# Kaixhin/imitation-learning

Measured on NVIDIA H100. Metric: env_steps_per_s, higher is better.
Workload: dtype f32

## Files before the change

imitation-learning_b200/csrc/api.cu:

```cuda
#include "common.cuh"
#include <cstdlib>

thread_local char g_il_error[512] = "";
int gail_init();
int gmmil_pwil_init();
int gemm_init();
int mlp_init();

extern "C" const char* il_last_error(void) { return g_il_error; }
extern "C" int il_version(void) { return 100; }

extern "C" int il_create(int device, il_handle** out) {
  IL_CHECK(out != nullptr, "il_create: null out");
  int count = 0;
  cudaError_t e = cudaGetDeviceCount(&count);
  if (e != cudaSuccess || count == 0) IL_FAIL("il_create: no CUDA device (%s); this library has no CPU fallback", cudaGetErrorString(e));
  IL_CHECK(device >= 0 && device < count, "il_create: device %d out of range (%d devices)", device, count);
  cudaDeviceProp prop;
  IL_CUDA(cudaGetDeviceProperties(&prop, device));
  IL_CHECK(prop.major == 9 && prop.minor == 0, "il_create: device %d is sm_%d%d; this library is built for sm_90a (H100) only", device, prop.major, prop.minor);
  IL_CUDA(cudaSetDevice(device));
  IL_TRY(gail_init());
  IL_TRY(gmmil_pwil_init());
  IL_TRY(tc_gemm_init());
  IL_TRY(gemm_init());
  IL_TRY(mlp_init());
  il_handle* h = new il_handle();
  h->device = device;
  h->sm_count = prop.multiProcessorCount;
  h->gemm_mode = IL_GEMM_FP32;
  {
    const char* wt = getenv("IL_WIDE_TN");
    h->wide_tn = (wt && wt[0] == '0') ? 0 : 1;
    const char* ff = getenv("IL_FIRST_LAYER_FAST");
    h->first_layer_fast = ff ? atoi(ff) : 2;
    const char* mb = getenv("IL_MASK_BITS");
    h->mask_bits = mb ? atoi(mb) : 2;
    const char* hf = getenv("IL_HEAD_FUSED");
    h->head_fused = (hf && hf[0] == '0') ? 0 : 1;
    const char* ds = getenv("IL_DEBUG_SYNC");
    h->debug_sync = (ds && ds[0] == '1') ? 1 : 0;
    const char* at = getenv("IL_ADAM_TMA");
    h->adam_tma = at ? atoi(at) : 1;
    const char* gt = getenv("IL_GAIL_TILED");
    h->gail_tiled = (gt && gt[0] == '0') ? 0 : 1;
    const char* fl = getenv("IL_TC_FUSE_L1");
    h->tc_fuse_l1 = (fl && fl[0] == '1') ? 1 : 0;
    const char* th = getenv("IL_THIN_HOIST");
    h->thin_hoist = (th && th[0] == '0') ? 0 : 1;
  }
  h->launches = 0;
  h->profiling = 0;
  h->profiled_bytes = 0.0;
  h->eval_graph = nullptr;
  h->build_stream = nullptr;
  *out = h;
  return 0;
}

extern "C" int il_destroy(il_handle* h) {
  if (h) il_eval_release(h);
  if (h && h->build_stream) cudaStreamDestroy(h->build_stream);
  delete h;
  return 0;
}

extern "C" int il_set_gemm_mode(il_handle* h, int mode) {
  IL_CHECK(h, "il_set_gemm_mode: null handle");
  IL_CHECK(mode >= IL_GEMM_FP32 && mode <= IL_GEMM_TF32, "il_set_gemm_mode: bad mode %d", mode);
  h->gemm_mode = mode;
  return 0;
}

extern "C" int64_t il_launch_count(il_handle* h) { return h ? h->launches : -1; }

extern "C" int il_set_option(il_handle* h, const char* name, int value) {
  IL_CHECK(h && name, "il_set_option: null argument");
  if (!strcmp(name, "tc_fuse_l1")) h->tc_fuse_l1 = value;
  else if (!strcmp(name, "gail_tiled")) h->gail_tiled = value;
  else if (!strcmp(name, "adam_tma")) h->adam_tma = value;
  else if (!strcmp(name, "head_fused")) h->head_fused = value;
  else if (!strcmp(name, "mask_bits")) h->mask_bits = value;
  else if (!strcmp(name, "first_layer_fast")) h->first_layer_fast = value;
  else if (!strcmp(name, "wide_tn")) h->wide_tn = value;
  else if (!strcmp(name, "thin_hoist")) h->thin_hoist = value;
  else IL_FAIL("il_set_option: unknown option '%s'", name);
  return 0;
}

extern "C" int il_struct_sizes(int32_t* out) {
  out[0] = (int32_t)sizeof(il_mlp);
  out[1] = (int32_t)sizeof(il_adam);
  out[2] = (int32_t)sizeof(il_batch);
  out[3] = (int32_t)sizeof(il_replay);
  out[4] = (int32_t)sizeof(il_sac_args);
  out[5] = (int32_t)sizeof(il_gail);
  out[6] = (int32_t)sizeof(il_gail_update_args);
  out[7] = (int32_t)sizeof(il_pwil);
  out[8] = (int32_t)sizeof(il_env);
  out[9] = (int32_t)sizeof(il_bc_args);
  out[10] = (int32_t)sizeof(il_eval_args);
  out[11] = (int32_t)sizeof(il_gailx);
  out[12] = (int32_t)sizeof(il_gailx_update_args);
  out[13] = (int32_t)sizeof(il_red);
  out[14] = (int32_t)sizeof(il_red_update_args);
  return 0;
}

extern "C" int il_mlp_param_offsets(const int32_t* dims, int n_layers, int64_t* w_off, int64_t* b_off, int64_t* total) {
  IL_CHECK(dims && n_layers >= 1 && n_layers <= IL_MAX_LAYERS, "il_mlp_param_offsets: bad arguments");
  const MlpOffsets o = mlp_offsets(dims, n_layers);
  for (int l = 0; l < n_layers; ++l) {
    if (w_off) w_off[l] = o.w[l];
    if (b_off) b_off[l] = o.b[l];
  }
  if (total) *total = o.total;
  return 0;
}

extern "C" int il_row_layout(int S, int A, int32_t* off, int32_t* row_len) {
  IL_CHECK(S > 0 && A > 0, "il_row_layout: S=%d A=%d", S, A);
  const RowLayout L = row_layout(S, A);
  if (off) {
    off[0] = L.state; off[1] = L.action; off[2] = L.reward; off[3] = L.next_state;
    off[4] = L.terminal; off[5] = L.timeout; off[6] = L.weight; off[7] = L.step;
  }
  if (row_len) *row_len = L.len;
  return 0;
}

namespace {

__global__ void fill_kernel(float* __restrict__ out, int64_t n, uint64_t seed, uint64_t stream_id, const uint64_t* __restrict__ counter, int normal,
                            const uint64_t* __restrict__ seed_r) {
  const uint64_t base = counter ? *counter : 0ull;
  if (seed_r) { seed = seed_r[blockIdx.y]; out += (int64_t)blockIdx.y * n; }
  const uint2 key = make_uint2((uint32_t)seed, (uint32_t)(seed >> 32));
  for (int64_t q = (int64_t)blockIdx.x * blockDim.x + threadIdx.x; q * 4 < n; q += (int64_t)gridDim.x * blockDim.x) {
    const uint64_t c = base + (uint64_t)q;
    const uint4 r = philox4x32_10(make_uint4((uint32_t)c, (uint32_t)(c >> 32), (uint32_t)stream_id, (uint32_t)(stream_id >> 32)), key);
    float v[4];
    if (normal) {
      const float u0 = 1.f - u32_to_unit(r.x), u1 = u32_to_unit(r.y), u2 = 1.f - u32_to_unit(r.z), u3 = u32_to_unit(r.w);
      const float r0 = sqrtf(-2.f * logf(u0)), r1 = sqrtf(-2.f * logf(u2));
      float s0, c0, s1, c1;
      sincospif(2.f * u1, &s0, &c0);
      sincospif(2.f * u3, &s1, &c1);
      v[0] = r0 * c0; v[1] = r0 * s0; v[2] = r1 * c1; v[3] = r1 * s1;
    } else {
      v[0] = u32_to_unit(r.x); v[1] = u32_to_unit(r.y); v[2] = u32_to_unit(r.z); v[3] = u32_to_unit(r.w);
    }
    for (int j = 0; j < 4; ++j)
      if (q * 4 + j < n) out[q * 4 + j] = v[j];
  }
}

constexpr int BETA_ATTEMPTS = 16;

__device__ float log_gamma_mt(float a, uint64_t c, uint64_t stream_id, uint32_t tag, uint2 key, float* boost_u) {
  const float d = a - 1.f / 3.f, cc = 1.f / sqrtf(9.f * d);
  for (int k = 0; k < BETA_ATTEMPTS; ++k) {
    const uint4 q = philox4x32_10(make_uint4((uint32_t)c, (uint32_t)(c >> 32), (uint32_t)stream_id, (uint32_t)(stream_id >> 32) ^ (tag | (uint32_t)k)), key);
    if (k == 0) *boost_u = 1.f - u32_to_unit(q.w);
    const float x = sqrtf(-2.f * logf(1.f - u32_to_unit(q.x))) * cospif(2.f * u32_to_unit(q.y));
    const float t = fmaf(cc, x, 1.f);
    if (t <= 0.f) continue;
    const float lt = logf(t), v = t * t * t;
    if (logf(1.f - u32_to_unit(q.z)) < 0.5f * x * x + d - d * v + 3.f * d * lt) return logf(d) + 3.f * lt;
  }
  return logf(d);
}

__global__ void beta_fill_kernel(float* __restrict__ out, int64_t total, int64_t n, const float* __restrict__ alpha_r, uint64_t seed, uint64_t stream_id,
                                 const uint64_t* __restrict__ counter, const uint64_t* __restrict__ seed_r) {
  const uint64_t base = counter ? *counter : 0ull;
  if (seed_r) { seed = seed_r[blockIdx.y]; out += (int64_t)blockIdx.y * n; total = n; }
  const uint2 key = make_uint2((uint32_t)seed, (uint32_t)(seed >> 32));
  for (int64_t i = (int64_t)blockIdx.x * blockDim.x + threadIdx.x; i < total; i += (int64_t)gridDim.x * blockDim.x) {
    const uint64_t c = base + (uint64_t)(i >> 2);
    const uint32_t lane = (uint32_t)(i & 3);
    const float alpha = alpha_r[seed_r ? (int64_t)blockIdx.y : i / n];
    float v;
    if (alpha == 1.f) {
      const uint4 q = philox4x32_10(make_uint4((uint32_t)c, (uint32_t)(c >> 32), (uint32_t)stream_id, (uint32_t)(stream_id >> 32)), key);
      v = u32_to_unit(lane == 0 ? q.x : lane == 1 ? q.y : lane == 2 ? q.z : q.w);
    } else if (!(alpha > 0.f)) {
      v = __int_as_float(0x7fc00000);
    } else {
      const float a = alpha < 1.f ? alpha + 1.f : alpha;
      float ux, uy;
      float lx = log_gamma_mt(a, c, stream_id, 0x80000000u | (lane << 5), key, &ux);
      float ly = log_gamma_mt(a, c, stream_id, 0x80000000u | (lane << 5) | 16u, key, &uy);
      if (alpha < 1.f) { lx += logf(ux) / alpha; ly += logf(uy) / alpha; }
      const float t = ly - lx;
      v = t >= 0.f ? 1.f / (1.f + expf(t)) : 1.f - 1.f / (1.f + expf(-t));
    }
    out[i] = v;
  }
}

__global__ void counter_add_kernel(uint64_t* c, uint64_t inc) { *c += inc; }

dim3 rng_grid(il_handle* h, int64_t units, int R) {
  int64_t blocks = (units + 255) / 256;
  const int64_t cap = (int64_t)h->sm_count * 16 / R;
  if (blocks > cap) blocks = cap;
  if (blocks < 1) blocks = 1;
  return dim3((unsigned)blocks, (unsigned)R);
}

int fill(il_handle* h, float* out, int64_t n, uint64_t seed, uint64_t stream_id, const uint64_t* counter, void* stream, int normal) {
  IL_CHECK(h && out && n >= 0, "il_fill: bad argument");
  if (n == 0) return 0;
  int64_t blocks = (n / 4 + 255) / 256;
  if (blocks > (int64_t)h->sm_count * 16) blocks = (int64_t)h->sm_count * 16;
  if (blocks < 1) blocks = 1;
  IL_LAUNCH(h, fill_kernel, (unsigned)blocks, 256, 0, (cudaStream_t)stream, out, n, seed, stream_id, counter, normal, nullptr);
  return 0;
}

int fill_r(il_handle* h, float* out, int R, int64_t n_per_replica, const uint64_t* seed_r, uint64_t stream_id, const uint64_t* counter, void* stream, int normal) {
  IL_CHECK(h && out && seed_r && R > 0 && R <= IL_MAX_GRID_Y && n_per_replica >= 0, "il_fill_%s_r: bad argument (R = %d)", normal ? "normal" : "uniform", R);
  if (n_per_replica == 0) return 0;
  IL_LAUNCH(h, fill_kernel, rng_grid(h, (n_per_replica + 3) / 4, R), 256, 0, (cudaStream_t)stream, out, n_per_replica, 0ull, stream_id, counter, normal, seed_r);
  return 0;
}

}

extern "C" int il_fill_normal(il_handle* h, float* out, int64_t n, uint64_t seed, uint64_t stream_id, const uint64_t* counter, void* stream) {
  return fill(h, out, n, seed, stream_id, counter, stream, 1);
}
extern "C" int il_fill_uniform(il_handle* h, float* out, int64_t n, uint64_t seed, uint64_t stream_id, const uint64_t* counter, void* stream) {
  return fill(h, out, n, seed, stream_id, counter, stream, 0);
}
extern "C" int il_fill_normal_r(il_handle* h, float* out, int R, int64_t n_per_replica, const uint64_t* seed_r, uint64_t stream_id, const uint64_t* counter, void* stream) {
  return fill_r(h, out, R, n_per_replica, seed_r, stream_id, counter, stream, 1);
}
extern "C" int il_fill_uniform_r(il_handle* h, float* out, int R, int64_t n_per_replica, const uint64_t* seed_r, uint64_t stream_id, const uint64_t* counter, void* stream) {
  return fill_r(h, out, R, n_per_replica, seed_r, stream_id, counter, stream, 0);
}
extern "C" int il_fill_beta(il_handle* h, float* out, int R, int64_t n_per_replica, const float* alpha_r, uint64_t seed, uint64_t stream_id, const uint64_t* counter,
                            void* stream) {
  IL_CHECK(h && out && alpha_r && R > 0 && n_per_replica >= 0, "il_fill_beta: bad argument");
  const int64_t total = (int64_t)R * n_per_replica;
  if (total == 0) return 0;
  int64_t blocks = (total + 255) / 256;
  if (blocks > (int64_t)h->sm_count * 16) blocks = (int64_t)h->sm_count * 16;
  IL_LAUNCH(h, beta_fill_kernel, (unsigned)blocks, 256, 0, (cudaStream_t)stream, out, total, n_per_replica, alpha_r, seed, stream_id, counter, nullptr);
  return 0;
}
extern "C" int il_fill_beta_r(il_handle* h, float* out, int R, int64_t n_per_replica, const float* alpha_r, const uint64_t* seed_r, uint64_t stream_id,
                              const uint64_t* counter, void* stream) {
  IL_CHECK(h && out && alpha_r && seed_r && R > 0 && R <= IL_MAX_GRID_Y && n_per_replica >= 0, "il_fill_beta_r: bad argument (R = %d)", R);
  if (n_per_replica == 0) return 0;
  IL_LAUNCH(h, beta_fill_kernel, rng_grid(h, n_per_replica, R), 256, 0, (cudaStream_t)stream, out, n_per_replica, n_per_replica, alpha_r, 0ull, stream_id, counter, seed_r);
  return 0;
}
extern "C" int il_counter_add(il_handle* h, uint64_t* counter, uint64_t inc, void* stream) {
  IL_CHECK(h && counter, "il_counter_add: null argument");
  IL_LAUNCH(h, counter_add_kernel, 1, 1, 0, (cudaStream_t)stream, counter, inc);
  return 0;
}
```

imitation-learning_b200/csrc/common.cuh:

```cuda
#pragma once
#include <cuda_runtime.h>
#include <stdint.h>
#include <stdio.h>
#include <string.h>

#include <vector>

#include "../../include/il_b200.h"

#define IL_MAX_GRID_Y 65535

struct ProfiledLaunch {
  cudaEvent_t start, stop;
  double flops;
  double bytes;
};
struct il_handle {
  int device;
  int sm_count;
  int gemm_mode;
  int thin_hoist;
  int wide_tn;
  int first_layer_fast;
  int mask_bits;
  int head_fused;
  int debug_sync;
  int adam_tma;
  int gail_tiled;
  int tc_fuse_l1;
  long long launches;
  int profiling;
  std::vector<ProfiledLaunch> profiled;
  double profiled_bytes;
  void* eval_graph;
  cudaStream_t build_stream;
};
void il_eval_release(il_handle* h);

extern thread_local char g_il_error[512];

#define IL_FAIL(...)                                     \
  do {                                                   \
    snprintf(g_il_error, sizeof(g_il_error), __VA_ARGS__); \
    return 1;                                            \
  } while (0)

#define IL_CHECK(cond, ...)        \
  do {                             \
    if (!(cond)) IL_FAIL(__VA_ARGS__); \
  } while (0)

#define IL_CUDA(expr)                                                                             \
  do {                                                                                            \
    cudaError_t _e = (expr);                                                                      \
    if (_e != cudaSuccess) IL_FAIL("%s failed: %s (%s:%d)", #expr, cudaGetErrorString(_e), __FILE__, __LINE__); \
  } while (0)

#define IL_LAUNCH(h, kernel, grid, block, smem, stream, ...)                                      \
  do {                                                                                            \
    kernel<<<(grid), (block), (smem), (cudaStream_t)(stream)>>>(__VA_ARGS__);                     \
    (h)->launches++;                                                                              \
    cudaError_t _e = cudaPeekAtLastError();                                                       \
    if (_e != cudaSuccess) IL_FAIL("launch of %s failed: %s (%s:%d)", #kernel, cudaGetErrorString(_e), __FILE__, __LINE__); \
  } while (0)

#define IL_TRY(expr)          \
  do {                        \
    int _r = (expr);          \
    if (_r != 0) return _r;   \
  } while (0)

__host__ __device__ static inline int64_t il_align_up(int64_t x, int64_t a) { return (x + a - 1) / a * a; }

struct RowLayout {
  int state, action, reward, next_state, terminal, timeout, weight, step, len;
};
__host__ __device__ inline RowLayout row_layout(int S, int A) {
  RowLayout L;
  L.state = 0;
  L.action = S;
  L.reward = S + A;
  L.next_state = S + A + 1;
  L.terminal = 2 * S + A + 1;
  L.timeout = L.terminal + 1;
  L.weight = L.terminal + 2;
  L.step = L.terminal + 3;
  L.len = (2 * S + A + 5 + 3) / 4 * 4;
  return L;
}

struct MlpOffsets {
  int64_t w[IL_MAX_LAYERS], b[IL_MAX_LAYERS], total;
};
__host__ __device__ static inline MlpOffsets mlp_offsets(const int32_t* dims, int n_layers) {
  MlpOffsets o;
  int64_t off = 0;
  for (int l = 0; l < n_layers; ++l) {
    o.w[l] = off;
    off = il_align_up(off + (int64_t)dims[l + 1] * dims[l], 4);
    o.b[l] = off;
    off = il_align_up(off + dims[l + 1], 4);
  }
  o.total = il_align_up(off, 32);
  return o;
}

__device__ __forceinline__ float act_apply(float x, int act) {
  if (act == IL_ACT_RELU) return fmaxf(x, 0.f);
  if (act == IL_ACT_TANH) return tanhf(x);
  return 1.f / (1.f + expf(-x));
}
__device__ __forceinline__ float act_grad_from_output(float y, int act) {
  if (act == IL_ACT_RELU) return y > 0.f ? 1.f : 0.f;
  if (act == IL_ACT_TANH) return 1.f - y * y;
  return y * (1.f - y);
}
__device__ __forceinline__ float softplusf(float x) {
  return x > 20.f ? x : log1pf(expf(x));
}
__device__ __forceinline__ float sigmoidf(float x) { return 1.f / (1.f + expf(-x)); }

__device__ __forceinline__ float warp_sum(float v) {
#pragma unroll
  for (int o = 16; o > 0; o >>= 1) v += __shfl_xor_sync(0xffffffffu, v, o);
  return v;
}
__device__ __forceinline__ float warp_max(float v) {
#pragma unroll
  for (int o = 16; o > 0; o >>= 1) v = fmaxf(v, __shfl_xor_sync(0xffffffffu, v, o));
  return v;
}
__device__ __forceinline__ float block_sum(float v, float* red) {
  const int lane = threadIdx.x & 31, warp = threadIdx.x >> 5, nw = (blockDim.x + 31) >> 5;
  v = warp_sum(v);
  __syncthreads();
  if (lane == 0) red[warp] = v;
  __syncthreads();
  float r = 0.f;
  if (warp == 0) {
    r = lane < nw ? red[lane] : 0.f;
    r = warp_sum(r);
    if (lane == 0) red[0] = r;
  }
  __syncthreads();
  return red[0];
}

__device__ __forceinline__ uint4 philox4x32_10(uint4 ctr, uint2 key) {
  const uint32_t M0 = 0xD2511F53u, M1 = 0xCD9E8D57u, W0 = 0x9E3779B9u, W1 = 0xBB67AE85u;
#pragma unroll
  for (int i = 0; i < 10; ++i) {
    const uint32_t hi0 = __umulhi(M0, ctr.x), lo0 = M0 * ctr.x;
    const uint32_t hi1 = __umulhi(M1, ctr.z), lo1 = M1 * ctr.z;
    ctr = make_uint4(hi1 ^ ctr.y ^ key.x, lo1, hi0 ^ ctr.w ^ key.y, lo0);
    key.x += W0;
    key.y += W1;
  }
  return ctr;
}
__device__ __forceinline__ float u32_to_unit(uint32_t x) { return (float)(x >> 8) * (1.0f / 16777216.0f); }

struct GemmArgs {
  const float* A;
  int64_t a_gs;
  int a_gdiv, lda, a_kmajor;
  const float* B;
  int64_t b_gs;
  int b_gdiv, ldb, b_kmajor;
  float* C;
  int64_t c_gs;
  int ldc;
  const float* bias;
  int64_t bias_gs;
  int act;
  const float* mask;
  int64_t mask_gs;
  int ldmask, mask_act;
  float* colsum;
  int64_t colsum_gs;
  int accumulate;
  int M, N, K, G;
  const uint32_t* mask_bits;
  int64_t mask_bits_gs;
  uint32_t* bits_out;
  int64_t bits_out_gs;
};
int launch_gemm(il_handle* h, const GemmArgs& a, cudaStream_t stream);
bool gemm_uses_tc(const il_handle* h, const GemmArgs& a);
bool gemm_first_layer_emits_bits(const il_handle* h, const GemmArgs& a);
double gemm_algorithmic_bytes(const GemmArgs& a, bool stores_c);
int profile_open(il_handle* h, ProfiledLaunch* pl, double flops, double bytes, cudaStream_t stream);
int profile_close(il_handle* h, ProfiledLaunch* pl, cudaStream_t stream);

bool tc_gemm_eligible(const GemmArgs& a);
int launch_tc_gemm(il_handle* h, const GemmArgs& a, cudaStream_t stream);
int tc_gemm_init();
struct TcFuseL1 {
  const float* x;
  int64_t x_gs;
  int x_gdiv, x_ld, x_k;
  const float* w1;
  const float* b1;
  int64_t gs;
  float* store;
  int64_t store_gs;
};
bool tc_head_fusable(const il_handle* h, const GemmArgs& a, int head_n);
bool tc_l1_fusable(const il_handle* h, const GemmArgs& a, int x_k);
bool tc_dx_head_fusable(const il_handle* h, const GemmArgs& a, int head_n);
int launch_tc_gemm_dx_head(il_handle* h, const GemmArgs& a, const float* w, int64_t w_gs, int w_ns, int head_n, float* out, int64_t out_gs, cudaStream_t stream);
int launch_tc_gemm_head(il_handle* h, const GemmArgs& a, const float* head_w, const float* head_b, int64_t head_gs, int head_n, float* head_out, int64_t head_out_gs, int store_c,
                        cudaStream_t stream, const TcFuseL1* l1 = nullptr);
```

imitation-learning_b200/csrc/mlp.cu:

```cuda
#include "mlp.cuh"

#include <math.h>

constexpr int HB_MAXN = 8;
struct HeadBwdArgs {
  const float* dout; int64_t dout_gs; int dout_gdiv, ld_dout;
  const float* w; int64_t w_gs;
  const float* y; int64_t y_gs;
  float* dz; int64_t dz_gs;
  float* dw; float* db; float* db_prev; int64_t g_gs;
  int n, H, Nh;
};
int launch_head_backward(il_handle* h, const HeadBwdArgs& a, int G, cudaStream_t stream);
int launch_head_dx_bits(il_handle* h, const HeadBwdArgs& a, const uint32_t* bits, int64_t bits_gs, int G, cudaStream_t stream);

int mlp_validate(const il_mlp* m, const char* what) {
  IL_CHECK(m != nullptr && m->params != nullptr, "%s: null mlp", what);
  IL_CHECK(m->n_layers >= 1 && m->n_layers <= IL_MAX_LAYERS, "%s: n_layers %d out of range", what, m->n_layers);
  IL_CHECK(m->activation >= 0 && m->activation <= 2, "%s: bad activation %d", what, m->activation);
  for (int l = 0; l <= m->n_layers; ++l) IL_CHECK(m->dims[l] > 0, "%s: dims[%d] = %d", what, l, m->dims[l]);
  const MlpOffsets o = mlp_offsets(m->dims, m->n_layers);
  IL_CHECK(m->stride >= o.total - 31 && m->stride % 4 == 0, "%s: stride %lld too small / unaligned for %lld parameters", what, (long long)m->stride, (long long)o.total);
  IL_CHECK((reinterpret_cast<uintptr_t>(m->params) & 15) == 0, "%s: params not 16-byte aligned", what);
  return 0;
}

int mlp_max_hidden(const il_mlp* m) {
  int mx = 1;
  for (int l = 1; l <= m->n_layers; ++l) mx = m->dims[l] > mx ? m->dims[l] : mx;
  return mx;
}

static int64_t mlp_bits_bytes(const il_mlp* m, int G, int n, int l) {
  return m->dims[l + 1] % 32 == 0 ? il_align_up((int64_t)G * n * (m->dims[l + 1] / 32) * 4, 256) : 0;
}

int64_t mlp_acts_bytes(const il_mlp* m, int G, int n) {
  int64_t b = 0;
  for (int l = 0; l + 1 < m->n_layers; ++l) b += il_align_up((int64_t)G * n * m->dims[l + 1] * 4, 256) + mlp_bits_bytes(m, G, n, l);
  return b;
}

char* mlp_acts_carve(const il_mlp* m, int G, int n, char* ws, MlpActs* acts) {
  for (int l = 0; l < IL_MAX_LAYERS; ++l) { acts->hid[l] = nullptr; acts->bits[l] = nullptr; acts->bits_valid[l] = false; }
  for (int l = 0; l + 1 < m->n_layers; ++l) {
    acts->hid[l] = reinterpret_cast<float*>(ws);
    ws += il_align_up((int64_t)G * n * m->dims[l + 1] * 4, 256);
    if (mlp_bits_bytes(m, G, n, l)) {
      acts->bits[l] = reinterpret_cast<uint32_t*>(ws);
      ws += mlp_bits_bytes(m, G, n, l);
    }
  }
  return ws;
}

int mlp_forward(il_handle* h, const il_mlp* m, int G, int n, MatView X, MlpActs& acts, float* out, int64_t out_gs, int ld_out, cudaStream_t stream, int keep) {
  const MlpOffsets o = mlp_offsets(m->dims, m->n_layers);
  const int L = m->n_layers;
  const bool keep_hidden = keep != MLP_KEEP_NONE;
  const bool want_bits = h->mask_bits && keep_hidden && m->activation == IL_ACT_RELU;
  for (int l = 0; l < IL_MAX_LAYERS; ++l) acts.bits_valid[l] = false;
  auto layer_args = [&](int l) {
    GemmArgs a{};
    if (l == 0) { a.A = X.ptr; a.a_gs = X.gs; a.a_gdiv = X.gdiv; a.lda = X.ld; }
    else { a.A = acts.hid[l - 1]; a.a_gs = (int64_t)n * m->dims[l]; a.a_gdiv = 1; a.lda = m->dims[l]; }
    a.a_kmajor = 1;
    a.B = m->params + o.w[l]; a.b_gs = m->stride; a.b_gdiv = 1; a.ldb = m->dims[l]; a.b_kmajor = 1;
    a.bias = m->params + o.b[l]; a.bias_gs = m->stride;
    if (l == L - 1) { a.C = out; a.c_gs = out_gs; a.ldc = ld_out; a.act = -1; }
    else { a.C = acts.hid[l]; a.c_gs = (int64_t)n * m->dims[l + 1]; a.ldc = m->dims[l + 1]; a.act = m->activation; }
    a.M = n; a.N = m->dims[l + 1]; a.K = m->dims[l]; a.G = G;
    return a;
  };
  const bool head_shape = L >= 2 && m->activation == IL_ACT_RELU && ld_out == m->dims[L] && out_gs == (int64_t)n * m->dims[L];
  for (int l = 0; l < L; ++l) {
    if (head_shape && l == L - 2) {
      GemmArgs a = layer_args(l);
      if (tc_head_fusable(h, a, m->dims[L])) {
        const bool bits = want_bits && keep == MLP_KEEP_MASKS && acts.bits[l] && m->dims[L] <= HB_MAXN;
        if (bits) { a.bits_out = acts.bits[l]; a.bits_out_gs = (int64_t)n * (m->dims[l + 1] / 32); acts.bits_valid[l] = true; }
        IL_TRY(launch_tc_gemm_head(h, a, m->params + o.w[L - 1], m->params + o.b[L - 1], m->stride, m->dims[L], out, out_gs, keep_hidden && !bits ? 1 : 0, stream));
        return 0;
      }
    }
    if (head_shape && l == 0 && L == 3) {
      GemmArgs a1 = layer_args(1);
      a1.A = nullptr; a1.a_gs = 0; a1.a_gdiv = 1; a1.lda = m->dims[1];
      if (tc_head_fusable(h, a1, m->dims[L]) && tc_l1_fusable(h, a1, m->dims[0])) {
        TcFuseL1 f{};
        f.x = X.ptr; f.x_gs = X.gs; f.x_gdiv = X.gdiv; f.x_ld = X.ld; f.x_k = m->dims[0];
        f.w1 = m->params + o.w[0]; f.b1 = m->params + o.b[0]; f.gs = m->stride;
        f.store = keep_hidden ? acts.hid[0] : nullptr; f.store_gs = (int64_t)n * m->dims[1];
        IL_TRY(launch_tc_gemm_head(h, a1, m->params + o.w[L - 1], m->params + o.b[L - 1], m->stride, m->dims[L], out, out_gs, keep_hidden ? 1 : 0, stream, &f));
        return 0;
      }
    }
    GemmArgs a = layer_args(l);
    if (want_bits && l + 1 < L && acts.bits[l] && gemm_first_layer_emits_bits(h, a)) {
      a.bits_out = acts.bits[l]; a.bits_out_gs = (int64_t)n * (m->dims[l + 1] / 32);
      acts.bits_valid[l] = true;
    }
    IL_TRY(launch_gemm(h, a, stream));
  }
  return 0;
}

static bool head_backward_eligible(const il_mlp* m, int n, int64_t grad_stride) {
  const int L = m->n_layers, H = m->dims[L - 1], Nh = m->dims[L];
  return m->activation == IL_ACT_RELU && Nh <= HB_MAXN && H % 4 == 0 && n <= 1024 && grad_stride % 4 == 0 && m->stride % 4 == 0;
}

int mlp_backward(il_handle* h, const il_mlp* m, int G, int n, MatView X, const MlpActs& acts, MatView dOut, float* grads, int64_t grad_stride,
                 float* dX, int64_t dx_gs, int ld_dx, int dx_col0, int dx_cols, float* tmpA, float* tmpB, cudaStream_t stream) {
  const MlpOffsets o = mlp_offsets(m->dims, m->n_layers);
  const int L = m->n_layers;
  MatView dZ = dOut;
  float* next_tmp = tmpA;
  bool bias_done = false;
  for (int l = L - 1; l >= 0; --l) {
    MatView Xin = l == 0 ? X : MatView{acts.hid[l - 1], (int64_t)n * m->dims[l], 1, m->dims[l]};
    if (l == L - 1 && l > 0 && grads && h->head_fused && head_backward_eligible(m, n, grad_stride)) {
      HeadBwdArgs a{};
      a.dout = dZ.ptr; a.dout_gs = dZ.gs; a.dout_gdiv = dZ.gdiv; a.ld_dout = dZ.ld;
      a.w = m->params + o.w[l]; a.w_gs = m->stride;
      a.y = acts.hid[l - 1]; a.y_gs = (int64_t)n * m->dims[l];
      a.dz = next_tmp; a.dz_gs = (int64_t)n * m->dims[l];
      a.dw = grads + o.w[l]; a.db = grads + o.b[l]; a.db_prev = grads + o.b[l - 1]; a.g_gs = grad_stride;
      a.n = n; a.H = m->dims[l]; a.Nh = m->dims[l + 1];
      IL_TRY(launch_head_backward(h, a, G, stream));
      dZ = MatView{next_tmp, (int64_t)n * m->dims[l], 1, m->dims[l]};
      next_tmp = next_tmp == tmpA ? tmpB : tmpA;
      bias_done = true;
      continue;
    }
    if (l == L - 1 && l > 0 && !grads && acts.bits_valid[l - 1] && m->dims[l + 1] <= HB_MAXN) {
      HeadBwdArgs a{};
      a.dout = dZ.ptr; a.dout_gs = dZ.gs; a.dout_gdiv = dZ.gdiv; a.ld_dout = dZ.ld;
      a.w = m->params + o.w[l]; a.w_gs = m->stride;
      a.dz = next_tmp; a.dz_gs = (int64_t)n * m->dims[l];
      a.n = n; a.H = m->dims[l]; a.Nh = m->dims[l + 1];
      IL_TRY(launch_head_dx_bits(h, a, acts.bits[l - 1], (int64_t)n * (m->dims[l] / 32), G, stream));
      dZ = MatView{next_tmp, (int64_t)n * m->dims[l], 1, m->dims[l]};
      next_tmp = next_tmp == tmpA ? tmpB : tmpA;
      continue;
    }
    if (grads) {
      GemmArgs a{};
      a.A = dZ.ptr; a.a_gs = dZ.gs; a.a_gdiv = dZ.gdiv; a.lda = dZ.ld; a.a_kmajor = 0;
      a.B = Xin.ptr; a.b_gs = Xin.gs; a.b_gdiv = Xin.gdiv; a.ldb = Xin.ld; a.b_kmajor = 0;
      a.C = grads + o.w[l]; a.c_gs = grad_stride; a.ldc = m->dims[l]; a.act = -1;
      if (!bias_done) { a.colsum = grads + o.b[l]; a.colsum_gs = grad_stride; }
      bias_done = false;
      a.M = m->dims[l + 1]; a.N = m->dims[l]; a.K = n; a.G = G;
      IL_TRY(launch_gemm(h, a, stream));
    }
    if (l > 0) {
      GemmArgs a{};
      a.A = dZ.ptr; a.a_gs = dZ.gs; a.a_gdiv = dZ.gdiv; a.lda = dZ.ld; a.a_kmajor = 1;
      a.B = m->params + o.w[l]; a.b_gs = m->stride; a.b_gdiv = 1; a.ldb = m->dims[l]; a.b_kmajor = 0;
      a.C = next_tmp; a.c_gs = (int64_t)n * m->dims[l]; a.ldc = m->dims[l]; a.act = -1;
      a.mask_act = m->activation;
      a.M = n; a.N = m->dims[l]; a.K = m->dims[l + 1]; a.G = G;
      if (acts.bits_valid[l - 1] && m->activation == IL_ACT_RELU && gemm_uses_tc(h, a)) {
        a.mask_bits = acts.bits[l - 1]; a.mask_bits_gs = (int64_t)n * (m->dims[l] / 32);
        if (h->mask_bits >= 2 && l == 1 && !grads && dX && ld_dx == dx_cols && dx_gs == (int64_t)n * dx_cols && tc_dx_head_fusable(h, a, dx_cols)) {
          a.C = nullptr;
          IL_TRY(launch_tc_gemm_dx_head(h, a, m->params + o.w[0] + dx_col0, m->stride, m->dims[0], dx_cols, dX, dx_gs, stream));
          return 0;
        }
      } else {
        a.mask = acts.hid[l - 1]; a.mask_gs = (int64_t)n * m->dims[l]; a.ldmask = m->dims[l];
      }
      IL_TRY(launch_gemm(h, a, stream));
      dZ = MatView{next_tmp, (int64_t)n * m->dims[l], 1, m->dims[l]};
      next_tmp = next_tmp == tmpA ? tmpB : tmpA;
    } else if (dX) {
      GemmArgs a{};
      a.A = dZ.ptr; a.a_gs = dZ.gs; a.a_gdiv = dZ.gdiv; a.lda = dZ.ld; a.a_kmajor = 1;
      a.B = m->params + o.w[0] + dx_col0; a.b_gs = m->stride; a.b_gdiv = 1; a.ldb = m->dims[0]; a.b_kmajor = 0;
      a.C = dX; a.c_gs = dx_gs; a.ldc = ld_dx; a.act = -1;
      a.M = n; a.N = dx_cols; a.K = m->dims[1]; a.G = G;
      IL_TRY(launch_gemm(h, a, stream));
    }
  }
  return 0;
}

namespace {

__global__ void actor_head_kernel(const HeadFwdArgs p) {
  const int64_t row = (int64_t)blockIdx.x * blockDim.x + threadIdx.x;
  if (row >= (int64_t)p.R * p.n) return;
  const int r = (int)(row / p.n), i = (int)(row % p.n);
  const int A = p.A;
  const float* hd = p.head + row * 2 * A;
  float* act_row = p.action ? p.action + (int64_t)r * p.action_rs + (int64_t)i * p.ld_action : nullptr;
  if (p.copy_src && act_row) {
    const float* src = p.copy_src + (int64_t)r * p.copy_rs + (int64_t)i * p.copy_ld;
    for (int j = 0; j < p.copy_cols; ++j) act_row[j - p.copy_cols] = __ldg(src + j);
  }
  const float keep = p.zero_mask ? 1.f - __ldg(p.zero_mask + (int64_t)r * p.zero_mask_rs + (int64_t)i * p.zero_mask_ld) : 1.f;
  const float LOG_SQRT_2PI = 0.91893853320467274178f, LOG2 = 0.69314718055994530942f;
  const float A_LO = (float)(-1.0 + 1e-6), A_HI = (float)(1.0 - 1e-6);
  float sum_ladj = 0.f, sum_nlp = 0.f;
  const bool want_lp = p.log_prob != nullptr && (p.eps != nullptr || p.given != nullptr);
  for (int j = 0; j < A; ++j) {
    const float mu = hd[j];
    const float ls = fminf(fmaxf(hd[A + j], -20.f), 2.f);
    if (p.mean) p.mean[row * A + j] = mu;
    if (p.log_std) p.log_std[row * A + j] = ls;
    float x, a;
    const float sd = expf(ls);
    if (p.given) {
      a = fminf(fmaxf(p.given[row * A + j], A_LO), A_HI);
      x = atanhf(a);
    } else if (p.eps) {
      x = __fadd_rn(mu, __fmul_rn(sd, p.eps[row * A + j]));
      a = tanhf(x);
    } else {
      x = mu;
      a = tanhf(mu);
    }
    if (act_row && !p.given) act_row[j] = keep * a;
    if (want_lp) {
      const float var = __fmul_rn(sd, sd);
      const float diff = __fsub_rn(x, mu);
      float nlp = __fdiv_rn(-__fmul_rn(diff, diff), __fmul_rn(2.f, var));
      nlp = __fsub_rn(__fsub_rn(nlp, logf(sd)), LOG_SQRT_2PI);
      const float ladj = __fmul_rn(2.f, __fsub_rn(__fsub_rn(LOG2, x), softplusf(__fmul_rn(-2.f, x))));
      sum_nlp += nlp;
      sum_ladj += ladj;
    }
  }
  if (want_lp) p.log_prob[row] = __fadd_rn(__fsub_rn(0.f, sum_ladj), sum_nlp);
}

struct SmallFwdArgs {
  il_mlp m;
  MlpOffsets o;
  const float* X;
  int64_t x_gs;
  int x_gdiv, ldx, n, maxd;
  float* out;
  int tanh_first;
};
template <int NR>
__global__ void __launch_bounds__(256) mlp_small_forward_kernel(const SmallFwdArgs p) {
  extern __shared__ __align__(16) float sm[];
  const int g = blockIdx.x, r0 = blockIdx.y * NR, tid = threadIdx.x, warp = tid >> 5, lane = tid & 31;
  const int nr = min(NR, p.n - r0), L = p.m.n_layers, maxd = p.maxd;
  float* bufs[2] = {sm, sm + NR * maxd};
  const float* X = p.X + (int64_t)(g / p.x_gdiv) * p.x_gs;
  for (int idx = tid; idx < NR * p.m.dims[0]; idx += 256) {
    const int r = idx / p.m.dims[0], k = idx % p.m.dims[0];
    bufs[0][r * maxd + k] = r < nr ? __ldg(X + (int64_t)(r0 + r) * p.ldx + k) : 0.f;
  }
  const float* prm = p.m.params + (int64_t)g * p.m.stride;
  __syncthreads();
  for (int l = 0; l < L; ++l) {
    const int in = p.m.dims[l], od = p.m.dims[l + 1];
    const float* W = prm + p.o.w[l];
    const float* bias = prm + p.o.b[l];
    const float* xin = bufs[l & 1];
    float* xout = bufs[(l + 1) & 1];
    const bool vec = (in % 4 == 0) && (p.m.stride % 4 == 0);
    if (NR == 1 && vec && in <= 16) {
      for (int o = tid; o < od; o += 256) {
        const float4* wr = reinterpret_cast<const float4*>(W + (int64_t)o * in);
        float4 w4[4];
#pragma unroll
        for (int q = 0; q < 4; ++q) w4[q] = 4 * q < in ? __ldg(wr + q) : make_float4(0.f, 0.f, 0.f, 0.f);
        float v = __ldg(bias + o);
#pragma unroll
        for (int q = 0; q < 4; ++q)
          if (4 * q < in) {
            const float4 x4 = *reinterpret_cast<const float4*>(xin + 4 * q);
            v = fmaf(w4[q].x, x4.x, fmaf(w4[q].y, x4.y, fmaf(w4[q].z, x4.z, fmaf(w4[q].w, x4.w, v))));
          }
        if (l < L - 1) v = act_apply(v, p.m.activation);
        xout[o] = v;
      }
      __syncthreads();
      continue;
    }
    if (NR == 1 && vec && in % 128 == 0 && in <= 256) {
      const int kv = in >> 7;
      float4 x4[2];
#pragma unroll
      for (int v = 0; v < 2; ++v) x4[v] = v < kv ? *reinterpret_cast<const float4*>(xin + v * 128 + lane * 4) : make_float4(0.f, 0.f, 0.f, 0.f);
      for (int o0 = warp * 8; o0 < od; o0 += 64) {
        float4 w4[8][2];
#pragma unroll
        for (int u = 0; u < 8; ++u)
#pragma unroll
          for (int v = 0; v < 2; ++v)
            w4[u][v] = (o0 + u < od && v < kv) ? __ldg(reinterpret_cast<const float4*>(W + (int64_t)(o0 + u) * in + v * 128 + lane * 4)) : make_float4(0.f, 0.f, 0.f, 0.f);
        float a8[8];
#pragma unroll
        for (int u = 0; u < 8; ++u) {
          float t = 0.f;
#pragma unroll
          for (int v = 0; v < 2; ++v) t = fmaf(w4[u][v].x, x4[v].x, fmaf(w4[u][v].y, x4[v].y, fmaf(w4[u][v].z, x4[v].z, fmaf(w4[u][v].w, x4[v].w, t))));
          a8[u] = warp_sum(t);
        }
        if (lane < 8 && o0 + lane < od) {
          float v = a8[0];
#pragma unroll
          for (int u = 1; u < 8; ++u) v = lane == u ? a8[u] : v;
          v += __ldg(bias + o0 + lane);
          if (l < L - 1) v = act_apply(v, p.m.activation);
          xout[o0 + lane] = v;
        }
      }
      __syncthreads();
      continue;
    }
    if (NR == 1 && vec) {
      for (int o0 = warp * 4; o0 < od; o0 += 32) {
        float a4[4] = {0.f, 0.f, 0.f, 0.f};
        for (int k = lane * 4; k < in; k += 128) {
          const float4 x4 = *reinterpret_cast<const float4*>(xin + k);
          float4 w4[4];
#pragma unroll
          for (int u = 0; u < 4; ++u) w4[u] = o0 + u < od ? __ldg(reinterpret_cast<const float4*>(W + (int64_t)(o0 + u) * in + k)) : make_float4(0.f, 0.f, 0.f, 0.f);
#pragma unroll
          for (int u = 0; u < 4; ++u) a4[u] = fmaf(w4[u].x, x4.x, fmaf(w4[u].y, x4.y, fmaf(w4[u].z, x4.z, fmaf(w4[u].w, x4.w, a4[u]))));
        }
#pragma unroll
        for (int u = 0; u < 4; ++u) a4[u] = warp_sum(a4[u]);
        if (lane < 4 && o0 + lane < od) {
          float v = (lane == 0 ? a4[0] : lane == 1 ? a4[1] : lane == 2 ? a4[2] : a4[3]) + __ldg(bias + o0 + lane);
          if (l < L - 1) v = act_apply(v, p.m.activation);
          xout[o0 + lane] = v;
        }
      }
      __syncthreads();
      continue;
    }
    for (int o = warp; o < od; o += 8) {
      float acc[NR];
#pragma unroll
      for (int r = 0; r < NR; ++r) acc[r] = 0.f;
      const float* wr = W + (int64_t)o * in;
      if (vec) {
        for (int k = lane * 4; k < in; k += 128) {
          const float4 w4 = __ldg(reinterpret_cast<const float4*>(wr + k));
#pragma unroll
          for (int r = 0; r < NR; ++r) {
            const float4 x4 = *reinterpret_cast<const float4*>(xin + r * maxd + k);
            acc[r] = fmaf(w4.x, x4.x, fmaf(w4.y, x4.y, fmaf(w4.z, x4.z, fmaf(w4.w, x4.w, acc[r]))));
          }
        }
      } else {
        for (int k = lane; k < in; k += 32) {
          const float w = __ldg(wr + k);
#pragma unroll
          for (int r = 0; r < NR; ++r) acc[r] = fmaf(w, xin[r * maxd + k], acc[r]);
        }
      }
#pragma unroll
      for (int r = 0; r < NR; ++r) acc[r] = warp_sum(acc[r]);
      if (lane == 0) {
        const float b = __ldg(bias + o);
#pragma unroll
        for (int r = 0; r < NR; ++r) {
          float v = acc[r] + b;
          if (l < L - 1) v = act_apply(v, p.m.activation);
          xout[r * maxd + o] = v;
        }
      }
    }
    __syncthreads();
  }
  const int od = p.m.dims[L];
  const float* fin = bufs[L & 1];
  if (p.tanh_first > 0) {
    const int A = p.tanh_first;
    for (int idx = tid; idx < nr * A; idx += 256) {
      const int r = idx / A, o = idx % A;
      p.out[((int64_t)g * p.n + r0 + r) * A + o] = tanhf(fin[r * maxd + o]);
    }
    return;
  }
  for (int idx = tid; idx < nr * od; idx += 256) {
    const int r = idx / od, o = idx % od;
    p.out[((int64_t)g * p.n + r0 + r) * od + o] = fin[r * maxd + o];
  }
}

struct AdamReplicas {
  const double* lr_r;
  const double* wd_r;
  const float* tau_r;
  int64_t rf;
  float inv_rf;
  int R;
};
struct AdamCoef { float step_size, decay, tau, one_minus_tau; };
constexpr int ADAM_MAX_REPLICAS = 2048;
__device__ __forceinline__ void adam_fill_table(AdamCoef* tab, const AdamReplicas& rp, double lr, double wd, double beta1_d, const int64_t* step, float tau) {
  if (!rp.R) return;
  const double bc1 = 1.0 - pow(beta1_d, (double)*step);
  for (int r = threadIdx.x; r < rp.R; r += blockDim.x) {
    const double l = rp.lr_r ? rp.lr_r[r] : lr, w = rp.wd_r ? rp.wd_r[r] : wd;
    const float t = rp.tau_r ? rp.tau_r[r] : tau;
    tab[r] = AdamCoef{(float)(l / bc1), w != 0.0 ? (float)(1.0 - l * w) : 1.f, t, (float)(1.0 - (double)t)};
  }
}
__device__ __forceinline__ int adam_replica(int64_t f, const AdamReplicas& rp) {
  int r = (int)((float)f * rp.inv_rf);
  if ((int64_t)r * rp.rf > f) --r;
  else if ((int64_t)(r + 1) * rp.rf <= f) ++r;
  return r;
}

__global__ void adam_kernel(float* __restrict__ p, const float* __restrict__ g, float* __restrict__ m, float* __restrict__ v, const int64_t* __restrict__ step,
                            double lr, double beta1_d, double beta2_d, double eps_d, double wd, int64_t n, float* __restrict__ target, float tau, float one_minus_tau,
                            const AdamReplicas rp) {
  extern __shared__ AdamCoef adam_tab[];
  __shared__ float s_step_size, s_bc2_sqrt;
  if (threadIdx.x == 0) {
    const double t = (double)*step;
    const double bc1 = 1.0 - pow(beta1_d, t), bc2 = 1.0 - pow(beta2_d, t);
    s_step_size = (float)(lr / bc1);
    s_bc2_sqrt = (float)sqrt(bc2);
  }
  adam_fill_table(adam_tab, rp, lr, wd, beta1_d, step, tau);
  __syncthreads();
  const float step_size = s_step_size, bc2_sqrt = s_bc2_sqrt;
  const float decay = (float)(1.0 - lr * wd), w1 = (float)(1.0 - beta1_d), w2 = (float)(1.0 - beta2_d);
  const float beta2 = (float)beta2_d, eps = (float)eps_d;
  const bool has_wd = wd != 0.0;
  auto upd = [&](float& pi, float& mi, float& vi, float gi, float ss, float dc, bool wdf) {
    if (wdf) pi = __fmul_rn(pi, dc);
    mi = __fadd_rn(mi, __fmul_rn(w1, __fsub_rn(gi, mi)));
    vi = __fadd_rn(__fmul_rn(vi, beta2), __fmul_rn(__fmul_rn(w2, gi), gi));
    const float denom = __fadd_rn(__fdiv_rn(sqrtf(vi), bc2_sqrt), eps);
    pi = __fadd_rn(pi, __fmul_rn(-ss, __fdiv_rn(mi, denom)));
  };
  const int64_t n4 = n >> 2;
  for (int64_t i = (int64_t)blockIdx.x * blockDim.x + threadIdx.x; i < n4; i += (int64_t)gridDim.x * blockDim.x) {
    float ss = step_size, dc = decay, ta = tau, omt = one_minus_tau;
    bool wdf = has_wd;
    if (rp.R) {
      const AdamCoef c = adam_tab[adam_replica(i << 2, rp)];
      ss = c.step_size; dc = c.decay; wdf = c.decay != 1.f; ta = c.tau; omt = c.one_minus_tau;
    }
    float4 pv = reinterpret_cast<float4*>(p)[i], mv = reinterpret_cast<float4*>(m)[i], vv = reinterpret_cast<float4*>(v)[i];
    const float4 gv = reinterpret_cast<const float4*>(g)[i];
    upd(pv.x, mv.x, vv.x, gv.x, ss, dc, wdf); upd(pv.y, mv.y, vv.y, gv.y, ss, dc, wdf); upd(pv.z, mv.z, vv.z, gv.z, ss, dc, wdf); upd(pv.w, mv.w, vv.w, gv.w, ss, dc, wdf);
    reinterpret_cast<float4*>(p)[i] = pv; reinterpret_cast<float4*>(m)[i] = mv; reinterpret_cast<float4*>(v)[i] = vv;
    if (target) {
      const float tau = ta, one_minus_tau = omt;
      float4 tv = reinterpret_cast<float4*>(target)[i];
      tv.x = __fadd_rn(__fmul_rn(tv.x, tau), __fmul_rn(one_minus_tau, pv.x)); tv.y = __fadd_rn(__fmul_rn(tv.y, tau), __fmul_rn(one_minus_tau, pv.y));
      tv.z = __fadd_rn(__fmul_rn(tv.z, tau), __fmul_rn(one_minus_tau, pv.z)); tv.w = __fadd_rn(__fmul_rn(tv.w, tau), __fmul_rn(one_minus_tau, pv.w));
      reinterpret_cast<float4*>(target)[i] = tv;
    }
  }
  for (int64_t i = (n4 << 2) + (int64_t)blockIdx.x * blockDim.x + threadIdx.x; i < n; i += (int64_t)gridDim.x * blockDim.x) {
    float pi = p[i], mi = m[i], vi = v[i];
    upd(pi, mi, vi, g[i], step_size, decay, has_wd);
    p[i] = pi; m[i] = mi; v[i] = vi;
    if (target) target[i] = __fadd_rn(__fmul_rn(target[i], tau), __fmul_rn(one_minus_tau, pi));
  }
}

constexpr int ADAM_STREAMS = 5;
constexpr int ADAM_CONSUMERS = 256;
template <int TILE, int STAGES> constexpr int adam_tma_smem() { return STAGES * ADAM_STREAMS * TILE * 4 + 2 * STAGES * 8 + 64; }
__device__ __forceinline__ void adam_mbar_wait(uint32_t bar, uint32_t parity) {
  asm volatile(
      "{\n\t.reg .pred q;\n\t"
      "ADAM_WAIT:\n\t"
      "mbarrier.try_wait.parity.shared::cta.b64 q, [%0], %1;\n\t"
      "@q bra ADAM_DONE;\n\t"
      "bra ADAM_WAIT;\n\t"
      "ADAM_DONE:\n\t}" ::"r"(bar), "r"(parity) : "memory");
}
template <int TILE, int STAGES>
__global__ void __launch_bounds__(ADAM_CONSUMERS + 32) adam_tma_kernel(float* __restrict__ p, const float* __restrict__ g, float* __restrict__ m, float* __restrict__ v,
                                                                      const int64_t* __restrict__ step, double lr, double beta1_d, double beta2_d, double eps_d, double wd, int64_t n,
                                                                      float* __restrict__ target, float tau, float one_minus_tau, const AdamReplicas rp) {
  extern __shared__ __align__(128) uint8_t adam_smem[];
  float* buf = reinterpret_cast<float*>(adam_smem);
  AdamCoef* tab = reinterpret_cast<AdamCoef*>(adam_smem + adam_tma_smem<TILE, STAGES>());
  const uint32_t smem0 = (uint32_t)__cvta_generic_to_shared(buf);
  const uint32_t full0 = smem0 + (uint32_t)(STAGES * ADAM_STREAMS * TILE * 4), done0 = full0 + 8u * STAGES;
  __shared__ float s_step_size, s_bc2_sqrt;
  const int tid = threadIdx.x;
  adam_fill_table(tab, rp, lr, wd, beta1_d, step, tau);
  if (tid == 0) {
    const double t = (double)*step;
    s_step_size = (float)(lr / (1.0 - pow(beta1_d, t)));
    s_bc2_sqrt = (float)sqrt(1.0 - pow(beta2_d, t));
    for (int s_ = 0; s_ < STAGES; ++s_) {
      asm volatile("mbarrier.init.shared::cta.b64 [%0], 1;" ::"r"(full0 + 8u * s_));
      asm volatile("mbarrier.init.shared::cta.b64 [%0], %1;" ::"r"(done0 + 8u * s_), "r"(ADAM_CONSUMERS));
    }
    asm volatile("fence.mbarrier_init.release.cluster;" ::: "memory");
  }
  __syncthreads();
  const int64_t n_tiles = (n + TILE - 1) / TILE;
  const int n_streams = target ? 5 : 4;
  auto tile_floats = [&](int64_t tile) { const int64_t left = n - tile * TILE; return (int)(left < TILE ? left : TILE); };
  const int64_t my_tiles = blockIdx.x < n_tiles ? (n_tiles - blockIdx.x + gridDim.x - 1) / gridDim.x : 0;
  if (tid >= ADAM_CONSUMERS) {
    if (tid != ADAM_CONSUMERS) return;
    auto issue_loads = [&](int64_t k) {
      const int64_t tile = blockIdx.x + k * gridDim.x;
      const int stage = (int)(k % STAGES);
      const uint32_t bytes = (uint32_t)tile_floats(tile) * 4u, bar = full0 + 8u * stage;
      asm volatile("mbarrier.arrive.expect_tx.shared::cta.b64 _, [%0], %1;" ::"r"(bar), "r"(bytes * (uint32_t)n_streams) : "memory");
      const float* src[5] = {p, g, m, v, target};
      for (int q = 0; q < n_streams; ++q)
        asm volatile("cp.async.bulk.shared::cluster.global.mbarrier::complete_tx::bytes [%0], [%1], %2, [%3];" ::"r"(smem0 + (uint32_t)((stage * ADAM_STREAMS + q) * TILE * 4)),
                     "l"(src[q] + tile * TILE), "r"(bytes), "r"(bar) : "memory");
    };
    for (int64_t k = 0; k < STAGES - 1 && k < my_tiles; ++k) issue_loads(k);
    for (int64_t k = 0; k < my_tiles; ++k) {
      const int stage = (int)(k % STAGES);
      const int64_t tile = blockIdx.x + k * gridDim.x;
      if (k + STAGES - 1 < my_tiles) {
        if (k > 0) asm volatile("cp.async.bulk.wait_group.read 0;" ::: "memory");
        issue_loads(k + STAGES - 1);
      }
      adam_mbar_wait(done0 + 8u * stage, (uint32_t)((k / STAGES) & 1));
      const uint32_t bytes = (uint32_t)tile_floats(tile) * 4u;
      float* dst[5] = {p, nullptr, m, v, target};
      for (int q = 0; q < n_streams; ++q) {
        if (!dst[q]) continue;
        asm volatile("cp.async.bulk.global.shared::cta.bulk_group [%0], [%1], %2;" ::"l"(dst[q] + tile * TILE), "r"(smem0 + (uint32_t)((stage * ADAM_STREAMS + q) * TILE * 4)), "r"(bytes)
                     : "memory");
      }
      asm volatile("cp.async.bulk.commit_group;" ::: "memory");
    }
    asm volatile("cp.async.bulk.wait_group 0;" ::: "memory");
    return;
  }
  const float step_size = s_step_size, bc2_sqrt = s_bc2_sqrt;
  const float decay = (float)(1.0 - lr * wd), w1 = (float)(1.0 - beta1_d), w2 = (float)(1.0 - beta2_d), beta2 = (float)beta2_d, eps = (float)eps_d;
  const bool has_wd = wd != 0.0;
  auto upd = [&](float& pi, float& mi, float& vi, float gi, float ss, float dc, bool wdf) {
    if (wdf) pi = __fmul_rn(pi, dc);
    mi = __fadd_rn(mi, __fmul_rn(w1, __fsub_rn(gi, mi)));
    vi = __fadd_rn(__fmul_rn(vi, beta2), __fmul_rn(__fmul_rn(w2, gi), gi));
    const float denom = __fadd_rn(__fdiv_rn(sqrtf(vi), bc2_sqrt), eps);
    pi = __fadd_rn(pi, __fmul_rn(-ss, __fdiv_rn(mi, denom)));
  };
  for (int64_t k = 0; k < my_tiles; ++k) {
    const int stage = (int)(k % STAGES);
    const int64_t tile = blockIdx.x + k * gridDim.x;
    adam_mbar_wait(full0 + 8u * stage, (uint32_t)((k / STAGES) & 1));
    const int nf4 = tile_floats(tile) >> 2;
    float4* sp = reinterpret_cast<float4*>(buf + (stage * ADAM_STREAMS + 0) * TILE);
    const float4* sg = reinterpret_cast<const float4*>(buf + (stage * ADAM_STREAMS + 1) * TILE);
    float4* smm = reinterpret_cast<float4*>(buf + (stage * ADAM_STREAMS + 2) * TILE);
    float4* sv = reinterpret_cast<float4*>(buf + (stage * ADAM_STREAMS + 3) * TILE);
    float4* stg = reinterpret_cast<float4*>(buf + (stage * ADAM_STREAMS + 4) * TILE);
    for (int i = tid; i < nf4; i += ADAM_CONSUMERS) {
      float ss = step_size, dc = decay, ta = tau, omt = one_minus_tau;
      bool wdf = has_wd;
      if (rp.R) {
        const AdamCoef c = tab[adam_replica(tile * TILE + 4 * i, rp)];
        ss = c.step_size; dc = c.decay; wdf = c.decay != 1.f; ta = c.tau; omt = c.one_minus_tau;
      }
      float4 pv = sp[i], mv = smm[i], vv = sv[i];
      const float4 gv = sg[i];
      upd(pv.x, mv.x, vv.x, gv.x, ss, dc, wdf); upd(pv.y, mv.y, vv.y, gv.y, ss, dc, wdf); upd(pv.z, mv.z, vv.z, gv.z, ss, dc, wdf); upd(pv.w, mv.w, vv.w, gv.w, ss, dc, wdf);
      sp[i] = pv; smm[i] = mv; sv[i] = vv;
      if (target) {
        const float tau = ta, one_minus_tau = omt;
        float4 tv = stg[i];
        tv.x = __fadd_rn(__fmul_rn(tv.x, tau), __fmul_rn(one_minus_tau, pv.x)); tv.y = __fadd_rn(__fmul_rn(tv.y, tau), __fmul_rn(one_minus_tau, pv.y));
        tv.z = __fadd_rn(__fmul_rn(tv.z, tau), __fmul_rn(one_minus_tau, pv.z)); tv.w = __fadd_rn(__fmul_rn(tv.w, tau), __fmul_rn(one_minus_tau, pv.w));
        stg[i] = tv;
      }
    }
    asm volatile("fence.proxy.async.shared::cta;" ::: "memory");
    asm volatile("mbarrier.arrive.shared::cta.b64 _, [%0];" ::"r"(done0 + 8u * stage) : "memory");
  }
}

template <int TILE, int STAGES>
static int launch_adam_tma(il_handle* h, int ctas_per_sm, float* params, const float* grads, const il_adam* opt, int64_t n, cudaStream_t stream, float* polyak_target, float polyak_factor,
                           const AdamReplicas& rp) {
  static bool attr_set = false;
  if (!attr_set) {
    IL_CUDA(cudaFuncSetAttribute(adam_tma_kernel<TILE, STAGES>, cudaFuncAttributeMaxDynamicSharedMemorySize, adam_tma_smem<TILE, STAGES>() + ADAM_MAX_REPLICAS * (int)sizeof(AdamCoef)));
    attr_set = true;
  }
  const size_t smem = (size_t)adam_tma_smem<TILE, STAGES>() + (size_t)rp.R * sizeof(AdamCoef);
  IL_LAUNCH(h, (adam_tma_kernel<TILE, STAGES>), h->sm_count * ctas_per_sm, ADAM_CONSUMERS + 32, smem, stream, params, grads, opt->m, opt->v, opt->step, opt->lr, opt->beta1,
            opt->beta2, opt->eps, opt->weight_decay, n, polyak_target, polyak_factor, (float)(1.0 - (double)polyak_factor), rp);
  return 0;
}
constexpr int ADAM_TMA_MIN_TILES = 4096;


template <int NH>
__global__ void __launch_bounds__(256, 2) head_backward_kernel(const HeadBwdArgs p) {
  extern __shared__ __align__(16) float hb_sm[];
  const int g = blockIdx.y, n0 = blockIdx.x * 256, tid = threadIdx.x, tc = tid & 63, tr = tid >> 6, col = n0 + tc * 4;
  float* dos = hb_sm;
  float* red = hb_sm + p.n * HB_MAXN;
  const float* dout = p.dout + (int64_t)(g / p.dout_gdiv) * p.dout_gs;
  const bool active = col < p.H;
  const float* Y = p.y + (int64_t)g * p.y_gs + col;
  float4 yv[4], yn[4];
  auto fetch = [&](float4 (&dst)[4], int b0) {
#pragma unroll
    for (int u = 0; u < 4; ++u) {
      const int b = b0 + 4 * u;
      dst[u] = (active && b < p.n) ? __ldg(reinterpret_cast<const float4*>(Y + (int64_t)b * p.H)) : make_float4(0.f, 0.f, 0.f, 0.f);
    }
  };
  fetch(yv, tr);
  for (int i = tid; i < p.n * HB_MAXN; i += 256) {
    const int b = i / HB_MAXN, j = i % HB_MAXN;
    dos[i] = j < p.Nh ? __ldg(dout + (int64_t)b * p.ld_dout + j) : 0.f;
  }
  float4 w[NH];
#pragma unroll
  for (int j = 0; j < NH; ++j) w[j] = (active && j < p.Nh) ? __ldg(reinterpret_cast<const float4*>(p.w + (int64_t)g * p.w_gs + (int64_t)j * p.H + col)) : make_float4(0.f, 0.f, 0.f, 0.f);
  __syncthreads();
  float4 dw[NH], cs = make_float4(0.f, 0.f, 0.f, 0.f);
#pragma unroll
  for (int j = 0; j < NH; ++j) dw[j] = make_float4(0.f, 0.f, 0.f, 0.f);
  if (active) {
    float* DZ = p.dz + (int64_t)g * p.dz_gs + col;
    for (int b0 = tr; b0 < p.n; b0 += 16) {
      fetch(yn, b0 + 16);
#pragma unroll
      for (int u = 0; u < 4; ++u) {
        const int b = b0 + 4 * u;
        if (b >= p.n) continue;
        float dj[NH];
        if (NH == 1) dj[0] = dos[b * HB_MAXN];
        else {
          const float4 d0 = *reinterpret_cast<const float4*>(dos + b * HB_MAXN), d1 = *reinterpret_cast<const float4*>(dos + b * HB_MAXN + 4);
          const float t[8] = {d0.x, d0.y, d0.z, d0.w, d1.x, d1.y, d1.z, d1.w};
#pragma unroll
          for (int j = 0; j < NH; ++j) dj[j] = t[j];
        }
        float4 z = make_float4(0.f, 0.f, 0.f, 0.f);
#pragma unroll
        for (int j = 0; j < NH; ++j) {
          z.x = fmaf(dj[j], w[j].x, z.x); z.y = fmaf(dj[j], w[j].y, z.y); z.z = fmaf(dj[j], w[j].z, z.z); z.w = fmaf(dj[j], w[j].w, z.w);
          dw[j].x = fmaf(dj[j], yv[u].x, dw[j].x); dw[j].y = fmaf(dj[j], yv[u].y, dw[j].y); dw[j].z = fmaf(dj[j], yv[u].z, dw[j].z); dw[j].w = fmaf(dj[j], yv[u].w, dw[j].w);
        }
        z.x = yv[u].x > 0.f ? z.x : 0.f; z.y = yv[u].y > 0.f ? z.y : 0.f; z.z = yv[u].z > 0.f ? z.z : 0.f; z.w = yv[u].w > 0.f ? z.w : 0.f;
        cs.x += z.x; cs.y += z.y; cs.z += z.z; cs.w += z.w;
        *reinterpret_cast<float4*>(DZ + (int64_t)b * p.H) = z;
      }
#pragma unroll
      for (int u = 0; u < 4; ++u) yv[u] = yn[u];
    }
  }
  float4* r4 = reinterpret_cast<float4*>(red);
#pragma unroll
  for (int j = 0; j < NH; ++j) r4[(tr * (HB_MAXN + 1) + j) * 64 + tc] = dw[j];
  r4[(tr * (HB_MAXN + 1) + HB_MAXN) * 64 + tc] = cs;
  __syncthreads();
  if (tr == 0 && active) {
#pragma unroll
    for (int j = 0; j <= HB_MAXN; ++j) {
      if ((j < NH && j < p.Nh) || j == HB_MAXN) {
        float4 a = r4[(0 * (HB_MAXN + 1) + j) * 64 + tc];
#pragma unroll
        for (int q = 1; q < 4; ++q) {
          const float4 t = r4[(q * (HB_MAXN + 1) + j) * 64 + tc];
          a.x += t.x; a.y += t.y; a.z += t.z; a.w += t.w;
        }
        float* dst = j == HB_MAXN ? p.db_prev + (int64_t)g * p.g_gs + col : p.dw + (int64_t)g * p.g_gs + (int64_t)j * p.H + col;
        *reinterpret_cast<float4*>(dst) = a;
      }
    }
  }
  if (blockIdx.x == 0 && tid < p.Nh) {
    float sacc = 0.f;
    for (int b = 0; b < p.n; ++b) sacc += dos[b * HB_MAXN + tid];
    p.db[(int64_t)g * p.g_gs + tid] = sacc;
  }
}

__global__ void tick_kernel(int64_t* s0, int64_t* s1, int64_t* s2) {
  if (s0) *s0 += 1;
  if (s1) *s1 += 1;
  if (s2) *s2 += 1;
}

__global__ void polyak_kernel(float* __restrict__ t, const float* __restrict__ o, int64_t n, float tau, float one_minus_tau) {
  for (int64_t i = (int64_t)blockIdx.x * blockDim.x + threadIdx.x; i < n; i += (int64_t)gridDim.x * blockDim.x)
    t[i] = __fadd_rn(__fmul_rn(t[i], tau), __fmul_rn(one_minus_tau, o[i]));
}

__global__ void split_twin_kernel(const float* __restrict__ q, float* __restrict__ q1, float* __restrict__ q2, int R, int n) {
  const int64_t i = (int64_t)blockIdx.x * blockDim.x + threadIdx.x;
  if (i >= (int64_t)R * n) return;
  const int r = (int)(i / n), b = (int)(i % n);
  if (q1) q1[i] = q[((int64_t)2 * r) * n + b];
  if (q2) q2[i] = q[((int64_t)2 * r + 1) * n + b];
}

__global__ void concat_kernel(const float* __restrict__ s, int64_t s_rs, int ld_s, int S, const float* __restrict__ a, int64_t a_rs, int ld_a, int A,
                              float* __restrict__ x, int R, int n) {
  const int64_t idx = (int64_t)blockIdx.x * blockDim.x + threadIdx.x;
  const int d = S + A;
  if (idx >= (int64_t)R * n * d) return;
  const int j = (int)(idx % d);
  const int64_t row = idx / d;
  const int r = (int)(row / n), i = (int)(row % n);
  x[idx] = j < S ? s[(int64_t)r * s_rs + (int64_t)i * ld_s + j] : a[(int64_t)r * a_rs + (int64_t)i * ld_a + (j - S)];
}

inline int ew_blocks(int64_t n, int threads, int sm_count) {
  int64_t b = (n + threads - 1) / threads;
  const int64_t cap = (int64_t)sm_count * 16;
  return (int)(b < 1 ? 1 : (b > cap ? cap : b));
}

}

int launch_actor_head(il_handle* h, const HeadFwdArgs& a, cudaStream_t stream) {
  const int64_t rows = (int64_t)a.R * a.n;
  IL_LAUNCH(h, actor_head_kernel, (unsigned)((rows + 127) / 128), 128, 0, stream, a);
  return 0;
}

int launch_adam(il_handle* h, float* params, const float* grads, const il_adam* opt, int64_t n, cudaStream_t stream, float* polyak_target, float polyak_factor,
                const float* polyak_r) {
  IL_CHECK(opt->m && opt->v && opt->step, "adam: null state");
  IL_CHECK(((reinterpret_cast<uintptr_t>(params) | reinterpret_cast<uintptr_t>(grads) | reinterpret_cast<uintptr_t>(opt->m) | reinterpret_cast<uintptr_t>(opt->v) |
             reinterpret_cast<uintptr_t>(polyak_target)) & 15) == 0, "adam: buffers must be 16-byte aligned");
  AdamReplicas rp{opt->lr_r, opt->weight_decay_r, polyak_target ? polyak_r : nullptr, 0, 0.f, 0};
  if (rp.lr_r || rp.wd_r || rp.tau_r) {
    const int64_t rf = opt->replica_floats;
    IL_CHECK(rf > 0 && rf % 4 == 0 && n % rf == 0, "adam: per-replica hyper-parameters need replica_floats (%lld) > 0, a multiple of 4 dividing n = %lld", (long long)rf, (long long)n);
    IL_CHECK(n / rf <= ADAM_MAX_REPLICAS, "adam: %lld replicas with per-replica hyper-parameters exceed the limit of %d per buffer", (long long)(n / rf), ADAM_MAX_REPLICAS);
    rp.rf = rf; rp.inv_rf = 1.f / (float)rf; rp.R = (int)(n / rf);
  }
  if (h->adam_tma && n % 4 == 0 && n >= (int64_t)ADAM_TMA_MIN_TILES * h->sm_count * 2) {
    const int variant = h->adam_tma;
    switch (variant) {
      case 2: return launch_adam_tma<4096, 2>(h, 1, params, grads, opt, n, stream, polyak_target, polyak_factor, rp);
      case 3: return launch_adam_tma<2048, 3>(h, 1, params, grads, opt, n, stream, polyak_target, polyak_factor, rp);
      case 4: return launch_adam_tma<1024, 4>(h, 2, params, grads, opt, n, stream, polyak_target, polyak_factor, rp);
      case 5: return launch_adam_tma<1024, 3>(h, 3, params, grads, opt, n, stream, polyak_target, polyak_factor, rp);
      case 6: return launch_adam_tma<512, 4>(h, 4, params, grads, opt, n, stream, polyak_target, polyak_factor, rp);
      case 7: return launch_adam_tma<2048, 4>(h, 1, params, grads, opt, n, stream, polyak_target, polyak_factor, rp);
      default: return launch_adam_tma<2048, 2>(h, 2, params, grads, opt, n, stream, polyak_target, polyak_factor, rp);
    }
  }
  IL_LAUNCH(h, adam_kernel, ew_blocks(n / 4 + 1, 256, h->sm_count), 256, (size_t)rp.R * sizeof(AdamCoef), stream, params, grads, opt->m, opt->v, opt->step, opt->lr, opt->beta1, opt->beta2,
            opt->eps, opt->weight_decay, n, polyak_target, polyak_factor, (float)(1.0 - (double)polyak_factor), rp);
  return 0;
}

namespace {
template <int NH, int U>
__global__ void __launch_bounds__(256) head_dx_bits_kernel(const HeadBwdArgs p, const uint32_t* __restrict__ bits, int64_t bits_gs) {
  const int g = blockIdx.y, tid = threadIdx.x, tc = tid & 63, tr = tid >> 6, col = blockIdx.x * 256 + tc * 4;
  if (col >= p.H) return;
  const float* __restrict__ dout = p.dout + (int64_t)(g / p.dout_gdiv) * p.dout_gs;
  const uint32_t* __restrict__ bw = bits + (int64_t)g * bits_gs + (col >> 5);
  const int sh = col & 31, wpr = p.H >> 5;
  float4 w[NH];
#pragma unroll
  for (int j = 0; j < NH; ++j) w[j] = j < p.Nh ? __ldg(reinterpret_cast<const float4*>(p.w + (int64_t)g * p.w_gs + (int64_t)j * p.H + col)) : make_float4(0.f, 0.f, 0.f, 0.f);
  float* __restrict__ dz = p.dz + (int64_t)g * p.dz_gs + col;
  for (int b0 = tr; b0 < p.n; b0 += 4 * U) {
    uint32_t m[U];
    float d[U][NH];
#pragma unroll
    for (int u = 0; u < U; ++u) {
      const int b = b0 + 4 * u;
      m[u] = b < p.n ? __ldg(bw + (int64_t)b * wpr) >> sh : 0u;
#pragma unroll
      for (int j = 0; j < NH; ++j) d[u][j] = (j < p.Nh && b < p.n) ? __ldg(dout + (int64_t)b * p.ld_dout + j) : 0.f;
    }
#pragma unroll
    for (int u = 0; u < U; ++u) {
      const int b = b0 + 4 * u;
      if (b >= p.n) break;
      float4 v = make_float4(0.f, 0.f, 0.f, 0.f);
#pragma unroll
      for (int j = 0; j < NH; ++j)
        if (j < p.Nh) { v.x = fmaf(d[u][j], w[j].x, v.x); v.y = fmaf(d[u][j], w[j].y, v.y); v.z = fmaf(d[u][j], w[j].z, v.z); v.w = fmaf(d[u][j], w[j].w, v.w); }
      v.x = m[u] & 1u ? v.x : 0.f; v.y = m[u] & 2u ? v.y : 0.f; v.z = m[u] & 4u ? v.z : 0.f; v.w = m[u] & 8u ? v.w : 0.f;
      *reinterpret_cast<float4*>(dz + (int64_t)b * p.H) = v;
    }
  }
}
}

int launch_head_dx_bits(il_handle* h, const HeadBwdArgs& a, const uint32_t* bits, int64_t bits_gs, int G, cudaStream_t stream) {
  IL_CHECK(a.H % 32 == 0 && a.Nh <= HB_MAXN && (reinterpret_cast<uintptr_t>(a.w) & 15) == 0 && a.w_gs % 4 == 0 && (reinterpret_cast<uintptr_t>(a.dz) & 15) == 0 && a.dz_gs % 4 == 0,
           "head_dx_bits: H=%d Nh=%d or unaligned buffers", a.H, a.Nh);
  if (a.Nh == 1) IL_LAUNCH(h, (head_dx_bits_kernel<1, 8>), dim3((a.H + 255) / 256, G), 256, 0, stream, a, bits, bits_gs);
  else IL_LAUNCH(h, (head_dx_bits_kernel<HB_MAXN, 4>), dim3((a.H + 255) / 256, G), 256, 0, stream, a, bits, bits_gs);
  return 0;
}

int launch_head_backward(il_handle* h, const HeadBwdArgs& a, int G, cudaStream_t stream) {
  const size_t smem = ((size_t)a.n * HB_MAXN + 4 * (HB_MAXN + 1) * 64 * 4) * sizeof(float);
  if (a.Nh == 1) IL_LAUNCH(h, head_backward_kernel<1>, dim3((a.H + 255) / 256, G), 256, smem, stream, a);
  else IL_LAUNCH(h, head_backward_kernel<HB_MAXN>, dim3((a.H + 255) / 256, G), 256, smem, stream, a);
  return 0;
}

int mlp_init() {
  IL_CUDA(cudaFuncSetAttribute(head_backward_kernel<1>, cudaFuncAttributeMaxDynamicSharedMemorySize, (1024 * HB_MAXN + 4 * (HB_MAXN + 1) * 64 * 4) * 4));
  IL_CUDA(cudaFuncSetAttribute(head_backward_kernel<HB_MAXN>, cudaFuncAttributeMaxDynamicSharedMemorySize, (1024 * HB_MAXN + 4 * (HB_MAXN + 1) * 64 * 4) * 4));
  return 0;
}

int launch_tick(il_handle* h, int64_t* s0, int64_t* s1, int64_t* s2, cudaStream_t stream) {
  IL_LAUNCH(h, tick_kernel, 1, 1, 0, stream, s0, s1, s2);
  return 0;
}

int mlp_small_forward(il_handle* h, const il_mlp* m, int G, int n, MatView X, float* out, cudaStream_t stream, int tanh_first) {
  SmallFwdArgs a;
  a.m = *m; a.o = mlp_offsets(m->dims, m->n_layers);
  a.X = X.ptr; a.x_gs = X.gs; a.x_gdiv = X.gdiv; a.ldx = X.ld; a.n = n; a.out = out; a.tanh_first = tanh_first;
  int maxd = 4;
  for (int l = 0; l <= m->n_layers; ++l) maxd = m->dims[l] > maxd ? m->dims[l] : maxd;
  a.maxd = (maxd + 3) / 4 * 4;
  if (n == 1) {
    IL_LAUNCH(h, mlp_small_forward_kernel<1>, dim3(G, 1), 256, (size_t)2 * 1 * a.maxd * 4, stream, a);
  } else {
    IL_CHECK((size_t)2 * 8 * a.maxd * 4 <= 48 * 1024, "mlp_small_forward: layer width %d too large", maxd);
    IL_LAUNCH(h, mlp_small_forward_kernel<8>, dim3(G, (n + 7) / 8), 256, (size_t)2 * 8 * a.maxd * 4, stream, a);
  }
  return 0;
}

extern "C" int il_adam_step(il_handle* h, float* params, const float* grads, const il_adam* opt, int64_t n, void* stream) {
  IL_CHECK(h && params && grads && opt, "il_adam_step: null argument");
  IL_TRY(launch_tick(h, opt->step, nullptr, nullptr, (cudaStream_t)stream));
  return launch_adam(h, params, grads, opt, n, (cudaStream_t)stream);
}

extern "C" int il_adam_step_polyak(il_handle* h, float* params, const float* grads, const il_adam* opt, int64_t n, float* target, float polyak_factor, void* stream) {
  IL_CHECK(h && params && grads && opt && target, "il_adam_step_polyak: null argument");
  IL_TRY(launch_tick(h, opt->step, nullptr, nullptr, (cudaStream_t)stream));
  return launch_adam(h, params, grads, opt, n, (cudaStream_t)stream, target, polyak_factor);
}

extern "C" int il_adam_step_polyak_r(il_handle* h, float* params, const float* grads, const il_adam* opt, int64_t n, float* target, const float* polyak_r, void* stream) {
  IL_CHECK(h && params && grads && opt && target && polyak_r, "il_adam_step_polyak_r: null argument");
  IL_TRY(launch_tick(h, opt->step, nullptr, nullptr, (cudaStream_t)stream));
  return launch_adam(h, params, grads, opt, n, (cudaStream_t)stream, target, 0.f, polyak_r);
}

extern "C" int il_polyak(il_handle* h, float* target, const float* online, int64_t n, float polyak_factor, void* stream) {
  IL_CHECK(h && target && online && n >= 0, "il_polyak: bad argument");
  if (n == 0) return 0;
  IL_LAUNCH(h, polyak_kernel, ew_blocks(n, 256, h->sm_count), 256, 0, (cudaStream_t)stream, target, online, n, polyak_factor, (float)(1.0 - (double)polyak_factor));
  return 0;
}

extern "C" int64_t il_actor_workspace_bytes(const il_mlp* actor, int R, int n) {
  return mlp_acts_bytes(actor, R, n) + il_align_up((int64_t)R * n * actor->dims[actor->n_layers] * 4, 256);
}

extern "C" int il_actor_forward(il_handle* h, const il_mlp* actor, int R, int n, const float* states, int64_t states_rs, int ld_states, const float* eps,
                                const float* given_action, float* action, float* log_prob, float* mean, float* log_std, void* workspace, int64_t workspace_bytes,
                                void* stream) {
  IL_CHECK(h && states && workspace, "il_actor_forward: null argument");
  IL_TRY(mlp_validate(actor, "il_actor_forward"));
  IL_CHECK(R > 0 && n > 0, "il_actor_forward: R=%d n=%d", R, n);
  const int out = actor->dims[actor->n_layers];
  IL_CHECK(out % 2 == 0, "il_actor_forward: head size %d is not 2*A", out);
  IL_CHECK(workspace_bytes >= il_actor_workspace_bytes(actor, R, n), "il_actor_forward: workspace too small");
  MlpActs acts;
  char* ws = mlp_acts_carve(actor, R, n, static_cast<char*>(workspace), &acts);
  float* head = reinterpret_cast<float*>(ws);
  if (n <= 32) IL_TRY(mlp_small_forward(h, actor, R, n, MatView{states, states_rs, 1, ld_states}, head, (cudaStream_t)stream));
  else IL_TRY(mlp_forward(h, actor, R, n, MatView{states, states_rs, 1, ld_states}, acts, head, (int64_t)n * out, out, (cudaStream_t)stream, MLP_KEEP_NONE));
  HeadFwdArgs a{};
  a.head = head; a.eps = eps; a.given = given_action;
  a.action = action; a.action_rs = (int64_t)n * (out / 2); a.ld_action = out / 2;
  a.log_prob = log_prob; a.mean = mean; a.log_std = log_std;
  a.R = R; a.n = n; a.A = out / 2;
  return launch_actor_head(h, a, (cudaStream_t)stream);
}

extern "C" int64_t il_critic_workspace_bytes(const il_mlp* critic, int R, int n) {
  return mlp_acts_bytes(critic, 2 * R, n) + il_align_up((int64_t)R * n * critic->dims[0] * 4, 256) + il_align_up((int64_t)2 * R * n * 4, 256);
}

extern "C" int il_critic_forward(il_handle* h, const il_mlp* twin, int R, int n, int S, const float* states, int64_t states_rs, int ld_states, const float* actions,
                                 int64_t actions_rs, int ld_actions, float* q1, float* q2, void* workspace, int64_t workspace_bytes, void* stream) {
  IL_CHECK(h && states && actions && workspace, "il_critic_forward: null argument");
  IL_TRY(mlp_validate(twin, "il_critic_forward"));
  IL_CHECK(twin->dims[twin->n_layers] == 1, "il_critic_forward: critic head must have one output");
  IL_CHECK(workspace_bytes >= il_critic_workspace_bytes(twin, R, n), "il_critic_forward: workspace too small");
  cudaStream_t st = (cudaStream_t)stream;
  const int d = twin->dims[0];
  MlpActs acts;
  char* ws = mlp_acts_carve(twin, 2 * R, n, static_cast<char*>(workspace), &acts);
  float* X = reinterpret_cast<float*>(ws);
  ws += il_align_up((int64_t)R * n * d * 4, 256);
  float* q = reinterpret_cast<float*>(ws);
  const int A = d - S;
  IL_CHECK(S > 0 && A > 0, "il_critic_forward: S=%d with input width %d", S, d);
  const int64_t total = (int64_t)R * n * d;
  IL_LAUNCH(h, concat_kernel, (unsigned)((total + 255) / 256), 256, 0, st, states, states_rs, ld_states, S, actions, actions_rs, ld_actions, A, X, R, n);
  IL_TRY(mlp_forward(h, twin, 2 * R, n, MatView{X, (int64_t)n * d, 2, d}, acts, q, (int64_t)n, 1, st, MLP_KEEP_NONE));
  IL_LAUNCH(h, split_twin_kernel, (unsigned)(((int64_t)R * n + 255) / 256), 256, 0, st, q, q1, q2, R, n);
  return 0;
}
```

imitation-learning_b200/csrc/mlp.cuh:

```cuda
#pragma once
#include "common.cuh"

struct MatView {
  const float* ptr;
  int64_t gs;
  int gdiv;
  int ld;
};

struct MlpActs {
  float* hid[IL_MAX_LAYERS];
  uint32_t* bits[IL_MAX_LAYERS];
  bool bits_valid[IL_MAX_LAYERS];
};
enum { MLP_KEEP_NONE = 0, MLP_KEEP_ALL = 1, MLP_KEEP_MASKS = 2 };

int64_t mlp_acts_bytes(const il_mlp* m, int G, int n);
char* mlp_acts_carve(const il_mlp* m, int G, int n, char* ws, MlpActs* acts);

int mlp_forward(il_handle* h, const il_mlp* m, int G, int n, MatView X, MlpActs& acts, float* out, int64_t out_gs, int ld_out,
                cudaStream_t stream, int keep = MLP_KEEP_ALL);

int mlp_backward(il_handle* h, const il_mlp* m, int G, int n, MatView X, const MlpActs& acts, MatView dOut, float* grads, int64_t grad_stride,
                 float* dX, int64_t dx_gs, int ld_dx, int dx_col0, int dx_cols, float* tmpA, float* tmpB, cudaStream_t stream);

int mlp_small_forward(il_handle* h, const il_mlp* m, int G, int n, MatView X, float* out, cudaStream_t stream, int tanh_first = 0);
int mlp_max_hidden(const il_mlp* m);
int mlp_validate(const il_mlp* m, const char* what);

struct HeadFwdArgs {
  const float* head;
  const float* eps;
  const float* given;
  float* action;
  int64_t action_rs;
  int ld_action;
  const float* zero_mask;
  int64_t zero_mask_rs;
  int zero_mask_ld;
  float* log_prob;
  float* mean;
  float* log_std;
  const float* copy_src;
  int64_t copy_rs;
  int copy_ld, copy_cols;
  int R, n, A;
};
int launch_actor_head(il_handle* h, const HeadFwdArgs& a, cudaStream_t stream);

int launch_adam(il_handle* h, float* params, const float* grads, const il_adam* opt, int64_t n, cudaStream_t stream, float* polyak_target = nullptr, float polyak_factor = 0.f,
                const float* polyak_r = nullptr);
int launch_tick(il_handle* h, int64_t* s0, int64_t* s1, int64_t* s2, cudaStream_t stream);
```

imitation-learning_b200/csrc/sac.cu:

```cuda
#include "mlp.cuh"

namespace {

struct AbsView {
  const float* ptr;
  int64_t rs;
  int ld;
};
__device__ __forceinline__ float abs_at(const AbsView& v, int r, int b) { return v.ptr ? __ldg(v.ptr + (int64_t)r * v.rs + (int64_t)b * v.ld) : 0.f; }

__global__ void sac_target_kernel(const float* __restrict__ qt, const float* __restrict__ lp_next, const float* __restrict__ log_alpha, const float* __restrict__ rows,
                                  int64_t rs, int row, int off_reward, int off_terminal, AbsView av, float discount, const float* __restrict__ discount_r, float* __restrict__ y,
                                  int R, int B) {
  const int64_t i = (int64_t)blockIdx.x * blockDim.x + threadIdx.x;
  if (i >= (int64_t)R * B) return;
  const int r = (int)(i / B), b = (int)(i % B);
  if (discount_r) discount = discount_r[r];
  const float alpha = expf(__ldg(log_alpha + r));
  const float* tr = rows + (int64_t)r * rs + (int64_t)b * row;
  const float q = fminf(qt[((int64_t)2 * r) * B + b], qt[((int64_t)2 * r + 1) * B + b]);
  const float ent = __fmul_rn(__fmul_rn(__fsub_rn(1.f, abs_at(av, r, b)), alpha), lp_next[i]);
  const float tv = __fsub_rn(q, ent);
  y[i] = __fadd_rn(tr[off_reward], __fmul_rn(__fmul_rn(__fsub_rn(1.f, tr[off_terminal]), discount), tv));
}

__global__ void sac_critic_lossgrad_kernel(const float* __restrict__ q, const float* __restrict__ y, const float* __restrict__ rows, int64_t rs, int row, int off_weight,
                                           float* __restrict__ dq, float* __restrict__ out_q, float* __restrict__ out_losses, int B) {
  __shared__ float red[32];
  const int r = blockIdx.x;
  const float invB = 1.f / (float)B;
  float l1 = 0.f, l2 = 0.f;
  for (int b = threadIdx.x; b < B; b += blockDim.x) {
    const float w = rows[(int64_t)r * rs + (int64_t)b * row + off_weight];
    const float yy = y[(int64_t)r * B + b];
    const float q1 = q[((int64_t)2 * r) * B + b], q2 = q[((int64_t)2 * r + 1) * B + b];
    const float d1 = __fsub_rn(q1, yy), d2 = __fsub_rn(q2, yy);
    l1 += w * d1 * d1;
    l2 += w * d2 * d2;
    const float c = __fmul_rn(invB, w);
    dq[((int64_t)2 * r) * B + b] = __fmul_rn(c, __fmul_rn(2.f, d1));
    dq[((int64_t)2 * r + 1) * B + b] = __fmul_rn(c, __fmul_rn(2.f, d2));
    if (out_q) out_q[(int64_t)r * B + b] = fminf(q1, q2);
  }
  l1 = block_sum(l1, red);
  l2 = block_sum(l2, red);
  if (threadIdx.x == 0 && out_losses) out_losses[r * 3 + 0] = l1 * invB + l2 * invB;
}

__global__ void sac_actor_loss_kernel(const float* __restrict__ q, const float* __restrict__ lp_new, const float* __restrict__ log_alpha, const float* __restrict__ rows,
                                      int64_t rs, int row, int off_weight, AbsView av, float* __restrict__ dq, float* __restrict__ out_losses, int B) {
  __shared__ float red[32];
  const int r = blockIdx.x;
  const float invB = 1.f / (float)B;
  const float alpha = expf(__ldg(log_alpha + r));
  float loss = 0.f;
  for (int b = threadIdx.x; b < B; b += blockDim.x) {
    const float w = rows[(int64_t)r * rs + (int64_t)b * row + off_weight];
    const float q1 = q[((int64_t)2 * r) * B + b], q2 = q[((int64_t)2 * r + 1) * B + b];
    const float g1 = q1 < q2 ? 1.f : (q1 == q2 ? 0.5f : 0.f);
    dq[((int64_t)2 * r) * B + b] = -invB * g1;
    dq[((int64_t)2 * r + 1) * B + b] = -invB * (1.f - g1);
    loss += w * (1.f - abs_at(av, r, b)) * alpha * lp_new[(int64_t)r * B + b] - fminf(q1, q2);
  }
  loss = block_sum(loss, red);
  if (threadIdx.x == 0 && out_losses) out_losses[r * 3 + 1] = loss * invB;
}

__global__ void sac_head_backward_kernel(const float* __restrict__ head, const float* __restrict__ eps, const float* __restrict__ xnew, int d, int S,
                                         const float* __restrict__ dxa, const float* __restrict__ log_alpha, const float* __restrict__ rows, int64_t rs, int row,
                                         int off_weight, AbsView av, float* __restrict__ dhead, int R, int B, int A) {
  const int64_t i = (int64_t)blockIdx.x * blockDim.x + threadIdx.x;
  if (i >= (int64_t)R * B) return;
  const int r = (int)(i / B), b = (int)(i % B);
  const float alpha = expf(__ldg(log_alpha + r));
  const float w = rows[(int64_t)r * rs + (int64_t)b * row + off_weight];
  const float c = w * (1.f - abs_at(av, r, b)) * alpha / (float)B;
  const float* hd = head + i * 2 * A;
  const float* a_row = xnew + i * d + S;
  const float* g1 = dxa + (((int64_t)2 * r) * B + b) * A;
  const float* g2 = dxa + (((int64_t)2 * r + 1) * B + b) * A;
  for (int j = 0; j < A; ++j) {
    const float raw = hd[A + j];
    const bool in_range = raw >= -20.f && raw <= 2.f;
    const float sd = expf(fminf(fmaxf(raw, -20.f), 2.f));
    const float a = a_row[j];
    const float dx = (g1[j] + g2[j]) * (1.f - a * a) + c * 2.f * a;
    dhead[i * 2 * A + j] = dx;
    dhead[i * 2 * A + A + j] = in_range ? dx * (sd * eps[i * A + j]) - c : 0.f;
  }
}

__global__ void sac_alpha_kernel(float* __restrict__ log_alpha, const float* __restrict__ lp_new, const float* __restrict__ rows, int64_t rs, int row, int off_weight,
                                 AbsView av, float entropy_target, const float* __restrict__ entropy_target_r, float* __restrict__ m, float* __restrict__ v,
                                 const int64_t* __restrict__ step, double lr, const double* __restrict__ lr_r, double beta1, double beta2, double eps, double wd,
                                 const double* __restrict__ wd_r, float* __restrict__ out_losses, int B) {
  __shared__ float red[32];
  const int r = blockIdx.x;
  if (entropy_target_r) entropy_target = entropy_target_r[r];
  if (lr_r) lr = lr_r[r];
  if (wd_r) wd = wd_r[r];
  float s = 0.f;
  for (int b = threadIdx.x; b < B; b += blockDim.x) {
    const float w = rows[(int64_t)r * rs + (int64_t)b * row + off_weight];
    s += w * (1.f - abs_at(av, r, b)) * (lp_new[(int64_t)r * B + b] + entropy_target);
  }
  s = block_sum(s, red);
  if (threadIdx.x == 0) {
    float p = log_alpha[r];
    const float alpha = expf(p);
    const float g = -alpha * s / (float)B;
    if (out_losses) out_losses[r * 3 + 2] = g;
    const double t = (double)*step;
    const float step_size = (float)(lr / (1.0 - pow(beta1, t))), bc2_sqrt = (float)sqrt(1.0 - pow(beta2, t));
    float mi = m[r], vi = v[r];
    if (wd != 0.0) p = __fmul_rn(p, (float)(1.0 - lr * wd));
    mi = __fadd_rn(mi, __fmul_rn((float)(1.0 - beta1), __fsub_rn(g, mi)));
    vi = __fadd_rn(__fmul_rn(vi, (float)beta2), __fmul_rn(__fmul_rn((float)(1.0 - beta2), g), g));
    const float denom = __fadd_rn(__fdiv_rn(sqrtf(vi), bc2_sqrt), (float)eps);
    p = __fadd_rn(p, __fmul_rn(-step_size, __fdiv_rn(mi, denom)));
    log_alpha[r] = p; m[r] = mi; v[r] = vi;
  }
}

__global__ void bc_head_backward_kernel(const float* __restrict__ head, const float* __restrict__ rows, int64_t rs, int row, int off_action, int off_weight,
                                        float* __restrict__ dhead, float* __restrict__ row_loss, int R, int B, int A) {
  const int64_t i = (int64_t)blockIdx.x * blockDim.x + threadIdx.x;
  if (i >= (int64_t)R * B) return;
  const int r = (int)(i / B), b = (int)(i % B);
  const float* tr = rows + (int64_t)r * rs + (int64_t)b * row;
  const float w = tr[off_weight], c = -w / (float)B;
  const float A_LO = (float)(-1.0 + 1e-6), A_HI = (float)(1.0 - 1e-6), LOG_SQRT_2PI = 0.91893853320467274178f, LOG2 = 0.69314718055994530942f;
  const float* hd = head + i * 2 * A;
  float lp = 0.f, ladj = 0.f;
  for (int j = 0; j < A; ++j) {
    const float raw = hd[A + j];
    const bool in_range = raw >= -20.f && raw <= 2.f;
    const float ls = fminf(fmaxf(raw, -20.f), 2.f), sd = expf(ls), var = sd * sd;
    const float x = atanhf(fminf(fmaxf(tr[off_action + j], A_LO), A_HI));
    const float diff = x - hd[j];
    lp += -(diff * diff) / (2.f * var) - logf(sd) - LOG_SQRT_2PI;
    ladj += 2.f * (LOG2 - x - softplusf(-2.f * x));
    dhead[i * 2 * A + j] = c * diff / var;
    dhead[i * 2 * A + A + j] = in_range ? c * (diff * diff / var - 1.f) : 0.f;
  }
  if (row_loss) row_loss[i] = -w * ((0.f - ladj) + lp);
}

__global__ void row_mean_kernel(const float* __restrict__ x, float* __restrict__ out, int B) {
  __shared__ float red[32];
  float s = 0.f;
  for (int b = threadIdx.x; b < B; b += blockDim.x) s += x[(int64_t)blockIdx.x * B + b];
  s = block_sum(s, red);
  if (threadIdx.x == 0) out[blockIdx.x] = s / (float)B;
}

struct SacWs {
  MlpActs actor_acts, critic_acts;
  float *head, *q, *xn, *y, *lp_next, *dq, *dxa, *dhead, *tmpA, *tmpB, *g_actor, *g_critic;
  int64_t bytes;
};

int64_t carve(char*& p, int64_t floats) {
  const int64_t b = il_align_up(floats * 4, 256);
  p += b;
  return b;
}

SacWs sac_layout(const il_sac_args* a, char* base) {
  SacWs w{};
  const int R = a->R, B = a->batch.B, A = a->batch.A, d = a->batch.S + a->batch.A;
  char* p = base;
  p = mlp_acts_carve(&a->actor, R, B, p, &w.actor_acts);
  p = mlp_acts_carve(&a->critic, 2 * R, B, p, &w.critic_acts);
  auto take = [&](int64_t floats) { float* r = reinterpret_cast<float*>(p); carve(p, floats); return r; };
  w.head = take((int64_t)R * B * 2 * A);
  w.q = take((int64_t)2 * R * B);
  w.xn = take((int64_t)R * B * d);
  w.y = take((int64_t)R * B);
  w.lp_next = take((int64_t)R * B);
  w.dq = take((int64_t)2 * R * B);
  w.dxa = take((int64_t)2 * R * B * A);
  w.dhead = take((int64_t)R * B * 2 * A);
  int hmax = mlp_max_hidden(&a->critic);
  if (mlp_max_hidden(&a->actor) > hmax) hmax = mlp_max_hidden(&a->actor);
  w.tmpA = take((int64_t)2 * R * B * hmax);
  w.tmpB = take((int64_t)2 * R * B * hmax);
  w.g_actor = take((int64_t)R * a->actor.stride);
  w.g_critic = take((int64_t)2 * R * a->critic.stride);
  w.bytes = p - base;
  return w;
}

}

extern "C" int64_t il_sac_workspace_bytes(const il_sac_args* a) {
  if (!a) return -1;
  return sac_layout(a, nullptr).bytes;
}

extern "C" int il_sac_update(il_handle* h, const il_sac_args* a, void* stream) {
  IL_CHECK(h && a, "il_sac_update: null argument");
  cudaStream_t st = (cudaStream_t)stream;
  const int R = a->R, B = a->batch.B, S = a->batch.S, A = a->batch.A, d = S + A;
  IL_CHECK(R > 0 && B > 0 && S > 0 && A > 0, "il_sac_update: R=%d B=%d S=%d A=%d", R, B, S, A);
  IL_TRY(mlp_validate(&a->actor, "il_sac_update(actor)"));
  IL_TRY(mlp_validate(&a->critic, "il_sac_update(critic)"));
  IL_TRY(mlp_validate(&a->target, "il_sac_update(target)"));
  IL_CHECK(a->actor.dims[0] == S && a->actor.dims[a->actor.n_layers] == 2 * A, "il_sac_update: actor dims do not match S=%d A=%d", S, A);
  IL_CHECK(a->critic.dims[0] == d && a->critic.dims[a->critic.n_layers] == 1, "il_sac_update: critic dims do not match S+A=%d", d);
  IL_CHECK(a->target.n_layers == a->critic.n_layers && a->target.stride == a->critic.stride, "il_sac_update: target/critic layout mismatch");
  const RowLayout L = row_layout(S, A);
  IL_CHECK(a->batch.row == L.len, "il_sac_update: batch row length %d != %d", a->batch.row, L.len);
  IL_CHECK(a->batch.rows && a->log_alpha && a->eps_next && a->eps_new && a->workspace, "il_sac_update: null buffer");
  IL_CHECK(a->workspace_bytes >= il_sac_workspace_bytes(a), "il_sac_update: workspace too small (%lld < %lld)", (long long)a->workspace_bytes,
           (long long)il_sac_workspace_bytes(a));
  IL_CHECK(!(a->actor_opt.lr_r || a->actor_opt.weight_decay_r) || a->actor_opt.replica_floats == a->actor.stride, "il_sac_update: actor_opt.replica_floats must be the actor stride");
  IL_CHECK(!(a->critic_opt.lr_r || a->critic_opt.weight_decay_r || a->polyak_r) || a->critic_opt.replica_floats == 2 * a->critic.stride,
           "il_sac_update: critic_opt.replica_floats must be 2 x the critic stride");
  SacWs w = sac_layout(a, static_cast<char*>(a->workspace));
  const float* rows = a->batch.rows;
  const int64_t rs = a->batch.replica_stride;
  const int row = L.len;
  AbsView av{nullptr, 0, 0};
  if (a->absorbing) av = AbsView{a->absorbing, (int64_t)B, 1};
  else if (a->absorbing_from_state) av = AbsView{rows + L.state + (S - 1), rs, row};
  const unsigned ew = (unsigned)(((int64_t)R * B + 127) / 128);

  IL_TRY(launch_tick(h, a->actor_opt.step, a->critic_opt.step, a->alpha_opt.step, st));

  IL_TRY(mlp_forward(h, &a->actor, R, B, MatView{rows + L.next_state, rs, 1, row}, w.actor_acts, w.head, (int64_t)B * 2 * A, 2 * A, st, false));
  {
    HeadFwdArgs ha{};
    ha.head = w.head; ha.eps = a->eps_next;
    ha.action = w.xn + S; ha.action_rs = (int64_t)B * d; ha.ld_action = d;
    ha.zero_mask = av.ptr; ha.zero_mask_rs = av.rs; ha.zero_mask_ld = av.ld;
    ha.log_prob = w.lp_next;
    ha.copy_src = rows + L.next_state; ha.copy_rs = rs; ha.copy_ld = row; ha.copy_cols = S;
    ha.R = R; ha.n = B; ha.A = A;
    IL_TRY(launch_actor_head(h, ha, st));
  }
  IL_TRY(mlp_forward(h, &a->target, 2 * R, B, MatView{w.xn, (int64_t)B * d, 2, d}, w.critic_acts, w.q, (int64_t)B, 1, st, false));
  IL_LAUNCH(h, sac_target_kernel, ew, 128, 0, st, w.q, w.lp_next, a->log_alpha, rows, rs, row, L.reward, L.terminal, av, a->discount, a->discount_r, w.y, R, B);
  IL_TRY(mlp_forward(h, &a->critic, 2 * R, B, MatView{rows + L.state, rs, 2, row}, w.critic_acts, w.q, (int64_t)B, 1, st));
  IL_LAUNCH(h, sac_critic_lossgrad_kernel, R, 256, 0, st, w.q, w.y, rows, rs, row, L.weight, w.dq, a->out_q_values, a->out_losses, B);
  IL_TRY(mlp_backward(h, &a->critic, 2 * R, B, MatView{rows + L.state, rs, 2, row}, w.critic_acts, MatView{w.dq, (int64_t)B, 1, 1}, w.g_critic, a->critic.stride, nullptr, 0,
                      0, 0, 0, w.tmpA, w.tmpB, st));
  IL_TRY(launch_adam(h, a->critic.params, w.g_critic, &a->critic_opt, (int64_t)2 * R * a->critic.stride, st, a->target.params, a->polyak_factor, a->polyak_r));
  IL_TRY(mlp_forward(h, &a->actor, R, B, MatView{rows + L.state, rs, 1, row}, w.actor_acts, w.head, (int64_t)B * 2 * A, 2 * A, st));
  {
    HeadFwdArgs ha{};
    ha.head = w.head; ha.eps = a->eps_new;
    ha.action = w.xn + S; ha.action_rs = (int64_t)B * d; ha.ld_action = d;
    ha.log_prob = a->out_log_probs ? a->out_log_probs : w.lp_next;
    ha.copy_src = rows + L.state; ha.copy_rs = rs; ha.copy_ld = row; ha.copy_cols = S;
    ha.R = R; ha.n = B; ha.A = A;
    IL_TRY(launch_actor_head(h, ha, st));
  }
  const float* lp_new = a->out_log_probs ? a->out_log_probs : w.lp_next;
  IL_TRY(mlp_forward(h, &a->critic, 2 * R, B, MatView{w.xn, (int64_t)B * d, 2, d}, w.critic_acts, w.q, (int64_t)B, 1, st, MLP_KEEP_MASKS));
  IL_LAUNCH(h, sac_actor_loss_kernel, R, 256, 0, st, w.q, lp_new, a->log_alpha, rows, rs, row, L.weight, av, w.dq, a->out_losses, B);
  IL_TRY(mlp_backward(h, &a->critic, 2 * R, B, MatView{w.xn, (int64_t)B * d, 2, d}, w.critic_acts, MatView{w.dq, (int64_t)B, 1, 1}, nullptr, 0, w.dxa, (int64_t)B * A, A, S,
                      A, w.tmpA, w.tmpB, st));
  IL_LAUNCH(h, sac_head_backward_kernel, ew, 128, 0, st, w.head, a->eps_new, w.xn, d, S, w.dxa, a->log_alpha, rows, rs, row, L.weight, av, w.dhead, R, B, A);
  IL_TRY(mlp_backward(h, &a->actor, R, B, MatView{rows + L.state, rs, 1, row}, w.actor_acts, MatView{w.dhead, (int64_t)B * 2 * A, 1, 2 * A}, w.g_actor, a->actor.stride,
                      nullptr, 0, 0, 0, 0, w.tmpA, w.tmpB, st));
  IL_TRY(launch_adam(h, a->actor.params, w.g_actor, &a->actor_opt, (int64_t)R * a->actor.stride, st));
  IL_LAUNCH(h, sac_alpha_kernel, R, 256, 0, st, a->log_alpha, lp_new, rows, rs, row, L.weight, av, a->entropy_target, a->entropy_target_r, a->alpha_opt.m, a->alpha_opt.v,
            a->alpha_opt.step, a->alpha_opt.lr, a->alpha_opt.lr_r, a->alpha_opt.beta1, a->alpha_opt.beta2, a->alpha_opt.eps, a->alpha_opt.weight_decay, a->alpha_opt.weight_decay_r,
            a->out_losses, B);
  return 0;
}

namespace {
struct BcWs {
  MlpActs acts;
  float *head, *dhead, *row_loss, *tmpA, *tmpB, *grads;
  int64_t bytes;
};
BcWs bc_layout(const il_bc_args* a, char* base) {
  BcWs w{};
  const int R = a->R, B = a->batch.B, A = a->batch.A;
  char* p = mlp_acts_carve(&a->actor, R, B, base, &w.acts);
  auto take = [&](int64_t floats) { float* r = reinterpret_cast<float*>(p); carve(p, floats); return r; };
  w.head = take((int64_t)R * B * 2 * A);
  w.dhead = take((int64_t)R * B * 2 * A);
  w.row_loss = take((int64_t)R * B);
  const int hmax = mlp_max_hidden(&a->actor);
  w.tmpA = take((int64_t)R * B * hmax);
  w.tmpB = take((int64_t)R * B * hmax);
  w.grads = take((int64_t)R * a->actor.stride);
  w.bytes = p - base;
  return w;
}
}

int bc_head_backward_launch(il_handle* h, const float* head, const il_batch* batch, float* dhead, float* row_loss, int R, cudaStream_t st) {
  const RowLayout L = row_layout(batch->S, batch->A);
  IL_LAUNCH(h, bc_head_backward_kernel, (unsigned)(((int64_t)R * batch->B + 127) / 128), 128, 0, st, head, batch->rows, batch->replica_stride, L.len, L.action, L.weight, dhead, row_loss, R,
            batch->B, batch->A);
  return 0;
}
int bc_row_mean_launch(il_handle* h, const float* row_loss, float* out_loss, int R, int B, cudaStream_t st) {
  IL_LAUNCH(h, row_mean_kernel, R, 256, 0, st, row_loss, out_loss, B);
  return 0;
}

extern "C" int64_t il_bc_workspace_bytes(const il_bc_args* a) { return a ? bc_layout(a, nullptr).bytes : -1; }

extern "C" int il_bc_update(il_handle* h, const il_bc_args* a, void* stream) {
  IL_CHECK(h && a, "il_bc_update: null argument");
  cudaStream_t st = (cudaStream_t)stream;
  const int R = a->R, B = a->batch.B, S = a->batch.S, A = a->batch.A;
  IL_TRY(mlp_validate(&a->actor, "il_bc_update(actor)"));
  IL_CHECK(R > 0 && B > 0 && a->actor.dims[0] == S && a->actor.dims[a->actor.n_layers] == 2 * A, "il_bc_update: actor dims do not match the batch");
  const RowLayout L = row_layout(S, A);
  IL_CHECK(a->batch.rows && a->batch.row == L.len && a->workspace && a->workspace_bytes >= il_bc_workspace_bytes(a), "il_bc_update: bad batch / workspace");
  BcWs w = bc_layout(a, static_cast<char*>(a->workspace));
  const MatView X{a->batch.rows + L.state, a->batch.replica_stride, 1, L.len};
  IL_TRY(launch_tick(h, a->opt.step, nullptr, nullptr, st));
  IL_TRY(mlp_forward(h, &a->actor, R, B, X, w.acts, w.head, (int64_t)B * 2 * A, 2 * A, st));
  IL_LAUNCH(h, bc_head_backward_kernel, (unsigned)(((int64_t)R * B + 127) / 128), 128, 0, st, w.head, a->batch.rows, a->batch.replica_stride, L.len, L.action, L.weight, w.dhead,
            a->out_loss ? w.row_loss : nullptr, R, B, A);
  if (a->out_loss) IL_LAUNCH(h, row_mean_kernel, R, 256, 0, st, w.row_loss, a->out_loss, B);
  IL_TRY(mlp_backward(h, &a->actor, R, B, X, w.acts, MatView{w.dhead, (int64_t)B * 2 * A, 1, 2 * A}, w.grads, a->actor.stride, nullptr, 0, 0, 0, 0, w.tmpA, w.tmpB, st));
  return launch_adam(h, a->actor.params, w.grads, &a->opt, (int64_t)R * a->actor.stride, st);
}
```

imitation-learning_b200/csrc/tc_gemm.cu:

```cuda
#include "common.cuh"
#include <cstdio>
#include <cstdlib>

namespace {

constexpr int BM = 128, BN = 256, BK = 16;
constexpr int PRODUCER_THREADS = 128, CONSUMER_THREADS = 256;
constexpr int THREADS = PRODUCER_THREADS + CONSUMER_THREADS;
constexpr int LAUNCH_REGS = 168;
constexpr int producer_regs(bool fuse) { return fuse ? 72 : 56; }
constexpr int consumer_regs(bool fuse) { return (THREADS * LAUNCH_REGS - PRODUCER_THREADS * producer_regs(fuse)) / CONSUMER_THREADS; }
static_assert(THREADS * LAUNCH_REGS <= 65536 && consumer_regs(false) % 8 == 0 && consumer_regs(true) % 8 == 0, "tc_gemm: setmaxnreg split");
constexpr int CONSUMER_BAR = 1, PRODUCER_BAR = 2;
constexpr int A_BYTES = BM * BK * 4, B_BYTES = BN * BK * 4;
constexpr int B_HI = 0, B_LO = B_BYTES;
constexpr int STAGE_BYTES = 2 * B_BYTES;
constexpr int N_STAGES = 3;
constexpr int RAW_STAGES = 3;
constexpr int A_STAGES = N_STAGES + RAW_STAGES;
constexpr int A_T_LD = BM + 8, A_T_BYTES = BK * A_T_LD * 4;
constexpr int a_slot_bytes(bool fuse) { return fuse ? A_BYTES : A_T_BYTES; }
constexpr int HEAD_MAX = 8;
constexpr int HEAD_BYTES = (BN + HEAD_MAX * BN) * 4;
constexpr int L1_MAXK = 16, L1_ROWS = 256;
constexpr int L1_W_BYTES = L1_ROWS * L1_MAXK * 4, L1_B_BYTES = L1_ROWS * 4, L1_X_BYTES = BM * L1_MAXK * 4;
constexpr int RAW_OFF = N_STAGES * STAGE_BYTES, A_OFF = RAW_OFF + RAW_STAGES * B_BYTES;
constexpr int head_off(bool fuse) { return A_OFF + A_STAGES * a_slot_bytes(fuse); }
constexpr int l1_off(bool fuse) { return head_off(fuse) + HEAD_BYTES; }
constexpr int BAR_BYTES = 64;
static_assert(2 * N_STAGES * 8 <= BAR_BYTES && BAR_BYTES + 512 - 16 <= 1024, "tc_gemm: mbarrier area");
constexpr int smem_bytes(bool fuse) { return 1024 + l1_off(fuse) + (fuse ? L1_W_BYTES + L1_B_BYTES + L1_X_BYTES : 0); }
static_assert(smem_bytes(false) <= 227 * 1024 && smem_bytes(true) <= 227 * 1024, "tc_gemm: shared memory over the 227 KB per-CTA limit");

__device__ __forceinline__ uint32_t smem_u32(const void* p) { return (uint32_t)__cvta_generic_to_shared(p); }
__device__ __forceinline__ void fence_proxy_async() { asm volatile("fence.proxy.async.shared::cta;" ::: "memory"); }
__device__ __forceinline__ void wgmma_fence() { asm volatile("wgmma.fence.sync.aligned;" ::: "memory"); }
__device__ __forceinline__ void wgmma_commit() { asm volatile("wgmma.commit_group.sync.aligned;" ::: "memory"); }
template <int N>
__device__ __forceinline__ void wgmma_wait() { asm volatile("wgmma.wait_group.sync.aligned %0;" ::"n"(N) : "memory"); }
__device__ __forceinline__ void cp_async16(uint32_t dst, const float* src) { asm volatile("cp.async.cg.shared.global [%0], [%1], 16;" ::"r"(dst), "l"(src) : "memory"); }
__device__ __forceinline__ void cp_async_commit() { asm volatile("cp.async.commit_group;" ::: "memory"); }
template <int N>
__device__ __forceinline__ void cp_async_wait() { asm volatile("cp.async.wait_group %0;" ::"n"(N) : "memory"); }
__device__ __forceinline__ void mbar_init(uint32_t bar, uint32_t count) { asm volatile("mbarrier.init.shared::cta.b64 [%0], %1;" ::"r"(bar), "r"(count) : "memory"); }
__device__ __forceinline__ void mbar_arrive(uint32_t bar) { asm volatile("mbarrier.arrive.shared::cta.b64 _, [%0];" ::"r"(bar) : "memory"); }
__device__ __forceinline__ void mbar_wait(uint32_t bar, uint32_t parity) {
  asm volatile(
      "{\n .reg .pred p;\n"
      "WAIT:\n mbarrier.try_wait.parity.shared::cta.b64 p, [%0], %1;\n"
      " @!p bra WAIT;\n}" ::"r"(bar), "r"(parity) : "memory");
}
template <int ID, int N>
__device__ __forceinline__ void named_bar_sync() { asm volatile("bar.sync %0, %1;" ::"n"(ID), "n"(N) : "memory"); }
template <int R>
__device__ __forceinline__ void setmaxnreg_dec() { asm volatile("setmaxnreg.dec.sync.aligned.u32 %0;" ::"n"(R)); }
template <int R>
__device__ __forceinline__ void setmaxnreg_inc() { asm volatile("setmaxnreg.inc.sync.aligned.u32 %0;" ::"n"(R)); }
__device__ __forceinline__ void wgmma_tf32(float (&d)[128], const uint32_t (&a)[4], uint64_t b_desc) {
  asm volatile(
      "wgmma.mma_async.sync.aligned.m64n256k8.f32.tf32.tf32 {"
      "%0, %1, %2, %3, %4, %5, %6, %7, %8, %9, %10, %11, %12, %13, %14, %15, "
      "%16, %17, %18, %19, %20, %21, %22, %23, %24, %25, %26, %27, %28, %29, %30, %31, "
      "%32, %33, %34, %35, %36, %37, %38, %39, %40, %41, %42, %43, %44, %45, %46, %47, "
      "%48, %49, %50, %51, %52, %53, %54, %55, %56, %57, %58, %59, %60, %61, %62, %63, "
      "%64, %65, %66, %67, %68, %69, %70, %71, %72, %73, %74, %75, %76, %77, %78, %79, "
      "%80, %81, %82, %83, %84, %85, %86, %87, %88, %89, %90, %91, %92, %93, %94, %95, "
      "%96, %97, %98, %99, %100, %101, %102, %103, %104, %105, %106, %107, %108, %109, %110, %111, "
      "%112, %113, %114, %115, %116, %117, %118, %119, %120, %121, %122, %123, %124, %125, %126, %127 "
      "}, {%128, %129, %130, %131}, %132, 1, 1, 1;"
      : "+f"(d[0]), "+f"(d[1]), "+f"(d[2]), "+f"(d[3]), "+f"(d[4]), "+f"(d[5]), "+f"(d[6]), "+f"(d[7]),
        "+f"(d[8]), "+f"(d[9]), "+f"(d[10]), "+f"(d[11]), "+f"(d[12]), "+f"(d[13]), "+f"(d[14]), "+f"(d[15]),
        "+f"(d[16]), "+f"(d[17]), "+f"(d[18]), "+f"(d[19]), "+f"(d[20]), "+f"(d[21]), "+f"(d[22]), "+f"(d[23]),
        "+f"(d[24]), "+f"(d[25]), "+f"(d[26]), "+f"(d[27]), "+f"(d[28]), "+f"(d[29]), "+f"(d[30]), "+f"(d[31]),
        "+f"(d[32]), "+f"(d[33]), "+f"(d[34]), "+f"(d[35]), "+f"(d[36]), "+f"(d[37]), "+f"(d[38]), "+f"(d[39]),
        "+f"(d[40]), "+f"(d[41]), "+f"(d[42]), "+f"(d[43]), "+f"(d[44]), "+f"(d[45]), "+f"(d[46]), "+f"(d[47]),
        "+f"(d[48]), "+f"(d[49]), "+f"(d[50]), "+f"(d[51]), "+f"(d[52]), "+f"(d[53]), "+f"(d[54]), "+f"(d[55]),
        "+f"(d[56]), "+f"(d[57]), "+f"(d[58]), "+f"(d[59]), "+f"(d[60]), "+f"(d[61]), "+f"(d[62]), "+f"(d[63]),
        "+f"(d[64]), "+f"(d[65]), "+f"(d[66]), "+f"(d[67]), "+f"(d[68]), "+f"(d[69]), "+f"(d[70]), "+f"(d[71]),
        "+f"(d[72]), "+f"(d[73]), "+f"(d[74]), "+f"(d[75]), "+f"(d[76]), "+f"(d[77]), "+f"(d[78]), "+f"(d[79]),
        "+f"(d[80]), "+f"(d[81]), "+f"(d[82]), "+f"(d[83]), "+f"(d[84]), "+f"(d[85]), "+f"(d[86]), "+f"(d[87]),
        "+f"(d[88]), "+f"(d[89]), "+f"(d[90]), "+f"(d[91]), "+f"(d[92]), "+f"(d[93]), "+f"(d[94]), "+f"(d[95]),
        "+f"(d[96]), "+f"(d[97]), "+f"(d[98]), "+f"(d[99]), "+f"(d[100]), "+f"(d[101]), "+f"(d[102]), "+f"(d[103]),
        "+f"(d[104]), "+f"(d[105]), "+f"(d[106]), "+f"(d[107]), "+f"(d[108]), "+f"(d[109]), "+f"(d[110]), "+f"(d[111]),
        "+f"(d[112]), "+f"(d[113]), "+f"(d[114]), "+f"(d[115]), "+f"(d[116]), "+f"(d[117]), "+f"(d[118]), "+f"(d[119]),
        "+f"(d[120]), "+f"(d[121]), "+f"(d[122]), "+f"(d[123]), "+f"(d[124]), "+f"(d[125]), "+f"(d[126]), "+f"(d[127])
      : "r"(a[0]), "r"(a[1]), "r"(a[2]), "r"(a[3]), "l"(b_desc));
}
__device__ __forceinline__ uint64_t make_desc(uint32_t smem_addr) {
  return (uint64_t)((smem_addr >> 4) & 0x3FFF) | ((uint64_t)1 << 16) | ((uint64_t)(512 >> 4) << 32) | ((uint64_t)2 << 62);
}
__device__ __forceinline__ uint32_t sw64(int r, int c) { return (uint32_t)((r >> 3) * 512 + (r & 7) * 64 + ((c ^ ((r >> 1) & 3)) << 4)); }
__device__ __forceinline__ void sts128(uint32_t addr, uint32_t x, uint32_t y, uint32_t z, uint32_t w) {
  asm volatile("st.shared.v4.b32 [%0], {%1, %2, %3, %4};" ::"r"(addr), "r"(x), "r"(y), "r"(z), "r"(w) : "memory");
}
__device__ __forceinline__ uint4 lds128(uint32_t addr) {
  uint4 v;
  asm volatile("ld.shared.v4.b32 {%0, %1, %2, %3}, [%4];" : "=r"(v.x), "=r"(v.y), "=r"(v.z), "=r"(v.w) : "r"(addr));
  return v;
}
__device__ __forceinline__ uint32_t lds32(uint32_t addr) {
  uint32_t v;
  asm volatile("ld.shared.b32 %0, [%1];" : "=r"(v) : "r"(addr));
  return v;
}
__device__ __forceinline__ void ldsm_x4(uint32_t addr, uint32_t (&v)[4]) {
  asm volatile("ldmatrix.sync.aligned.m8n8.x4.shared.b16 {%0, %1, %2, %3}, [%4];" : "=r"(v[0]), "=r"(v[1]), "=r"(v[2]), "=r"(v[3]) : "r"(addr));
}
__device__ __forceinline__ uint32_t hi_of(uint32_t x) { return x & 0xFFFFE000u; }
__device__ __forceinline__ uint32_t lo_of(uint32_t x) { return __float_as_uint(__uint_as_float(x) - __uint_as_float(x & 0xFFFFE000u)); }
__device__ __forceinline__ void split_reg(uint32_t x, uint32_t& hi, uint32_t& lo) {
  asm volatile("and.b32 %0, %2, 0xFFFFE000;\n\tsub.f32 %1, %2, %0;" : "=&r"(hi), "=r"(lo) : "r"(x));
}
__device__ __forceinline__ void store_chunk(uint32_t hi_tile, uint32_t lo_tile, uint32_t off, uint4 v, bool split) {
  sts128(hi_tile + off, hi_of(v.x), hi_of(v.y), hi_of(v.z), hi_of(v.w));
  if (split) sts128(lo_tile + off, lo_of(v.x), lo_of(v.y), lo_of(v.z), lo_of(v.w));
}
__device__ __forceinline__ void store_block_t(uint32_t hi_tile, uint32_t lo_tile, int c4, int kg, const uint4 (&v)[4], bool split) {
  uint4 q0 = make_uint4(v[0].x, v[1].x, v[2].x, v[3].x), q1 = make_uint4(v[0].y, v[1].y, v[2].y, v[3].y);
  uint4 q2 = make_uint4(v[0].z, v[1].z, v[2].z, v[3].z), q3 = make_uint4(v[0].w, v[1].w, v[2].w, v[3].w);
  const int s = (c4 >> 1) & 3;
  if (s & 1) { const uint4 t = q0; q0 = q1; q1 = q2; q2 = q3; q3 = t; }
  if (s & 2) { uint4 t = q0; q0 = q2; q2 = t; t = q1; q1 = q3; q3 = t; }
  store_chunk(hi_tile, lo_tile, sw64(4 * c4 + (s & 3), kg), q0, split);
  store_chunk(hi_tile, lo_tile, sw64(4 * c4 + ((s + 1) & 3), kg), q1, split);
  store_chunk(hi_tile, lo_tile, sw64(4 * c4 + ((s + 2) & 3), kg), q2, split);
  store_chunk(hi_tile, lo_tile, sw64(4 * c4 + ((s + 3) & 3), kg), q3, split);
}

struct TcParams {
  GemmArgs g;
  int tiles_m;
  int split;
  const float* head_w;
  const float* head_b;
  float* head_out;
  int64_t head_gs, head_out_gs;
  int head_n, store_c;
  int head_js, head_ns;
  TcFuseL1 l1;
};

template <int EPI, bool FUSE = false>
__global__ void __launch_bounds__(THREADS, 1) tc_gemm_kernel(const TcParams p) {
  extern __shared__ uint8_t smem_raw[];
  uint8_t* smem = reinterpret_cast<uint8_t*>((reinterpret_cast<uintptr_t>(smem_raw) + BAR_BYTES + 511) & ~(uintptr_t)511);
  float* head_s = reinterpret_cast<float*>(smem + head_off(FUSE));
  const uint32_t stage0 = smem_u32(smem), raw0 = stage0 + RAW_OFF, a0s = stage0 + A_OFF;
  const uint32_t full0 = stage0 - BAR_BYTES, empty0 = full0 + N_STAGES * 8;
  const uint32_t w1s = stage0 + l1_off(FUSE), b1s = w1s + L1_W_BYTES, xs = b1s + L1_B_BYTES;
  auto a_slot = [&](int q) { return a0s + (uint32_t)(q % A_STAGES) * (uint32_t)a_slot_bytes(FUSE); };
  const bool a_km = FUSE || p.g.a_kmajor != 0;

  const int tid = threadIdx.x, warp = tid >> 5, lane = tid & 31, wg = tid >> 7;
  const GemmArgs& g = p.g;
  const int nkb = g.K / BK, tiles_m = p.tiles_m;
  const int my_tiles = (g.G * tiles_m - (int)blockIdx.x + (int)gridDim.x - 1) / (int)gridDim.x;
  const int nq = my_tiles * nkb;
  auto tile_of = [&](int i) { return (int)blockIdx.x + i * (int)gridDim.x; };

  if (tid == 0) {
#pragma unroll
    for (int s = 0; s < N_STAGES; ++s) {
      mbar_init(full0 + 8 * s, PRODUCER_THREADS);
      mbar_init(empty0 + 8 * s, CONSUMER_THREADS);
    }
  }
  __syncthreads();

  if (wg == 0) {
    setmaxnreg_dec<producer_regs(FUSE)>();
    const bool b_km = g.b_kmajor != 0, split = p.split != 0;
    constexpr int MAP = 2 * PRODUCER_THREADS;
    const int pt = tid;

    auto copy_kb = [&](int q) {
      if (q < nq) {
        const int t = tile_of(q / nkb), kb = q % nkb, grp = t / tiles_m, m0 = (t % tiles_m) * BM;
        const float* A = g.A + (int64_t)(grp / g.a_gdiv) * g.a_gs;
        const float* Bg = g.B + (int64_t)(grp / g.b_gdiv) * g.b_gs;
        const uint32_t as = a_slot(q);
#pragma unroll
        for (int h = 0; h < 2; ++h) {
          const int v = pt + h * PRODUCER_THREADS, fr = v >> 2, fc = v & 3;
          const uint32_t raw = raw0 + (uint32_t)(q % RAW_STAGES) * B_BYTES + (uint32_t)v * 16u;
          if (!FUSE) {
            if (a_km) {
              const float* src = A + (int64_t)(m0 + fr) * g.lda + kb * BK + fc * 4;
              cp_async16(as + sw64(fr, fc), src);
              cp_async16(as + sw64(fr, fc) + 4096u, src + (int64_t)64 * g.lda);
            } else if (h == 0) {
              const int c4 = v & 31, kg = v >> 5;
              const float* src = A + (int64_t)(kb * BK + kg * 4) * g.lda + m0 + c4 * 4;
#pragma unroll
              for (int k = 0; k < 4; ++k) cp_async16(as + (uint32_t)(((kg * 4 + k) * A_T_LD + c4 * 4) * 4), src + (int64_t)k * g.lda);
            }
          }
          const float* src = b_km ? Bg + (int64_t)fr * g.ldb + kb * BK + fc * 4 : Bg + (int64_t)(kb * BK + (v >> 6) * 4) * g.ldb + (v & 63) * 4;
          const int64_t step = b_km ? (int64_t)64 * g.ldb : (int64_t)g.ldb;
#pragma unroll
          for (int j = 0; j < 4; ++j) cp_async16(raw + j * MAP * 16, src + j * step);
        }
      }
      cp_async_commit();
    };

    auto split_kb = [&](int q, int s) {
      const uint32_t st = stage0 + (uint32_t)s * STAGE_BYTES;
#pragma unroll(FUSE ? 1 : 2)
      for (int h = 0; h < 2; ++h) {
        const int v = pt + h * PRODUCER_THREADS, fr = v >> 2, fc = v & 3;
        const uint32_t raw = raw0 + (uint32_t)(q % RAW_STAGES) * B_BYTES + (uint32_t)v * 16u;
        const uint32_t km_off = sw64(fr, fc);
        if (FUSE) {
          const int kb = q % nkb, k0 = kb * BK + fc * 4;
          const uint4 bq = lds128(b1s + (uint32_t)k0 * 4u);
          float c0[4] = {__uint_as_float(bq.x), __uint_as_float(bq.y), __uint_as_float(bq.z), __uint_as_float(bq.w)};
          float c1[4] = {c0[0], c0[1], c0[2], c0[3]};
          const int np = (p.l1.x_k + 3) >> 2;
#pragma unroll
          for (int c4 = 0; c4 < L1_MAXK / 4; ++c4) {
            if (c4 < np) {
              const uint4 x0 = lds128(xs + sw64(fr, c4)), x1 = lds128(xs + sw64(fr + 64, c4));
#pragma unroll
              for (int qq = 0; qq < 4; ++qq) {
                const uint4 w = lds128(w1s + (uint32_t)((k0 + qq) * 64 + ((c4 ^ fc) << 4)));
                c0[qq] = fmaf(__uint_as_float(x0.x), __uint_as_float(w.x), c0[qq]); c1[qq] = fmaf(__uint_as_float(x1.x), __uint_as_float(w.x), c1[qq]);
                c0[qq] = fmaf(__uint_as_float(x0.y), __uint_as_float(w.y), c0[qq]); c1[qq] = fmaf(__uint_as_float(x1.y), __uint_as_float(w.y), c1[qq]);
                c0[qq] = fmaf(__uint_as_float(x0.z), __uint_as_float(w.z), c0[qq]); c1[qq] = fmaf(__uint_as_float(x1.z), __uint_as_float(w.z), c1[qq]);
                c0[qq] = fmaf(__uint_as_float(x0.w), __uint_as_float(w.w), c0[qq]); c1[qq] = fmaf(__uint_as_float(x1.w), __uint_as_float(w.w), c1[qq]);
              }
            }
          }
          const uint4 a0 = make_uint4(__float_as_uint(fmaxf(c0[0], 0.f)), __float_as_uint(fmaxf(c0[1], 0.f)), __float_as_uint(fmaxf(c0[2], 0.f)), __float_as_uint(fmaxf(c0[3], 0.f)));
          const uint4 a1 = make_uint4(__float_as_uint(fmaxf(c1[0], 0.f)), __float_as_uint(fmaxf(c1[1], 0.f)), __float_as_uint(fmaxf(c1[2], 0.f)), __float_as_uint(fmaxf(c1[3], 0.f)));
          const uint32_t as = a_slot(q);
          sts128(as + km_off, a0.x, a0.y, a0.z, a0.w);
          sts128(as + km_off + 4096u, a1.x, a1.y, a1.z, a1.w);
          if (p.l1.store) {
            const int t = tile_of(q / nkb);
            float* hs = p.l1.store + (int64_t)(t / tiles_m) * p.l1.store_gs + (int64_t)((t % tiles_m) * BM + fr) * g.K + k0;
            *reinterpret_cast<uint4*>(hs) = a0;
            *reinterpret_cast<uint4*>(hs + (int64_t)64 * g.K) = a1;
          }
        }
        if (b_km) {
#pragma unroll
          for (int j = 0; j < 4; ++j) store_chunk(st + B_HI, st + B_LO, km_off + (uint32_t)j * 4096u, lds128(raw + j * MAP * 16), split);
        } else {
          uint4 vb[4];
#pragma unroll
          for (int k = 0; k < 4; ++k) vb[k] = lds128(raw + k * MAP * 16);
          store_block_t(st + B_HI, st + B_LO, v & 63, v >> 6, vb, split);
        }
      }
    };

    auto stage_l1 = [&](int t) {
      const int grp = t / tiles_m, m0 = (t % tiles_m) * BM, xk = p.l1.x_k;
      const float* w1 = p.l1.w1 + (int64_t)grp * p.l1.gs;
      const float* b1 = p.l1.b1 + (int64_t)grp * p.l1.gs;
      const float* x = p.l1.x + (int64_t)(grp / p.l1.x_gdiv) * p.l1.x_gs + (int64_t)m0 * p.l1.x_ld;
      float* w1f = reinterpret_cast<float*>(smem + l1_off(FUSE));
      float* b1f = reinterpret_cast<float*>(smem + l1_off(FUSE) + L1_W_BYTES);
      float* xf = reinterpret_cast<float*>(smem + l1_off(FUSE) + L1_W_BYTES + L1_B_BYTES);
#pragma unroll 1
      for (int i = pt; i < L1_ROWS * L1_MAXK; i += PRODUCER_THREADS) {
        const int k = i / L1_MAXK, j = i % L1_MAXK;
        w1f[k * L1_MAXK + ((((j >> 2) ^ ((k >> 2) & 3)) << 2) | (j & 3))] = (k < g.K && j < xk) ? __ldg(w1 + (int64_t)k * xk + j) : 0.f;
      }
      for (int i = pt; i < L1_ROWS; i += PRODUCER_THREADS) b1f[i] = i < g.K ? __ldg(b1 + i) : 0.f;
#pragma unroll 1
      for (int i = pt; i < BM * L1_MAXK; i += PRODUCER_THREADS) {
        const int r = i / L1_MAXK, j = i % L1_MAXK;
        xf[(sw64(r, j >> 2) >> 2) + (j & 3)] = j < xk ? __ldg(x + (int64_t)r * p.l1.x_ld + j) : 0.f;
      }
    };

#pragma unroll 1
    for (int q = 0; q < RAW_STAGES; ++q) copy_kb(q);
    int s = 0;
    uint32_t ph = 1;
#pragma unroll 1
    for (int q = 0; q < nq; ++q) {
      if (FUSE && q % nkb == 0) {
        if (q > 0) named_bar_sync<PRODUCER_BAR, PRODUCER_THREADS>();
        stage_l1(tile_of(q / nkb));
        named_bar_sync<PRODUCER_BAR, PRODUCER_THREADS>();
      }
      mbar_wait(empty0 + 8 * s, ph);
      cp_async_wait<RAW_STAGES - 1>();
      split_kb(q, s);
      fence_proxy_async();
      mbar_arrive(full0 + 8 * s);
      copy_kb(q + RAW_STAGES);
      if (++s == N_STAGES) { s = 0; ph ^= 1; }
    }
    cp_async_wait<0>();
    return;
  }

  setmaxnreg_inc<consumer_regs(FUSE)>();
  const int cw = wg - 1, ct = tid - PRODUCER_THREADS;
  const uint64_t b_desc0 = make_desc(stage0);
  const bool split = p.split != 0;
  const int wrow = cw * 64 + (warp & 3) * 16, g8 = lane >> 2, t4 = lane & 3;
  const uint32_t lm_off = sw64(wrow + (lane & 7) + 8 * ((lane >> 3) & 1), lane >> 4);
  const uint32_t t_off = (uint32_t)((t4 * A_T_LD + wrow + g8) * 4);
  uint32_t af[2][2][BK / 8][4];
  float acc[128];
  auto kblock = [&](int q, int s, uint32_t (&f)[2][BK / 8][4]) {
    const uint32_t as = a_slot(q), cur = (uint32_t)s * STAGE_BYTES;
#pragma unroll
    for (int kk = 0; kk < BK / 8; ++kk) {
      uint32_t x[4];
      if (a_km) {
        ldsm_x4(as + (lm_off ^ (uint32_t)(kk * 32)), x);
      } else {
#pragma unroll
        for (int j = 0; j < 4; ++j) x[j] = lds32(as + t_off + (uint32_t)(((8 * kk + 4 * (j >> 1)) * A_T_LD + 8 * (j & 1)) * 4));
      }
#pragma unroll
      for (int j = 0; j < 4; ++j) split_reg(x[j], f[0][kk][j], f[1][kk][j]);
    }
    wgmma_fence();
#pragma unroll
    for (int kk = 0; kk < BK / 8; ++kk) {
      const uint32_t o = cur + kk * 32;
      const uint64_t bh = b_desc0 + ((o + B_HI) >> 4), bl = b_desc0 + ((o + B_LO) >> 4);
      if (split) {
        wgmma_tf32(acc, f[1][kk], bh);
        wgmma_tf32(acc, f[0][kk], bl);
      }
      wgmma_tf32(acc, f[0][kk], bh);
    }
    wgmma_commit();
  };
  int s = 0, q = 0;
  uint32_t ph = 0;
#pragma unroll 1
  for (int i = 0; i < my_tiles; ++i) {
#pragma unroll
    for (int j = 0; j < 128; ++j) acc[j] = 0.f;
    int prev = 0;
    auto step = [&](int kb, uint32_t (&f)[2][BK / 8][4]) {
      mbar_wait(full0 + 8 * s, ph);
      kblock(q, s, f);
      wgmma_wait<1>();
      if (kb > 0) mbar_arrive(empty0 + 8 * prev);
      prev = s;
      ++q;
      if (++s == N_STAGES) { s = 0; ph ^= 1; }
    };
#pragma unroll 1
    for (int kb = 0; kb < nkb; kb += 2) {
      step(kb, af[0]);
      if (kb + 1 < nkb) step(kb + 1, af[1]);
    }

    const int t = tile_of(i), grp = t / tiles_m, m0 = (t % tiles_m) * BM;
    if (EPI == 4 || EPI == 6) {
      named_bar_sync<CONSUMER_BAR, CONSUMER_THREADS>();
      const float* wsrc = p.head_w + (int64_t)grp * p.head_gs;
      if (EPI == 4) head_s[ct] = __ldg(g.bias + (int64_t)grp * g.bias_gs + ct);
#pragma unroll
      for (int j = 0; j < HEAD_MAX; ++j)
        if (j < p.head_n) head_s[BN + j * BN + ct] = __ldg(wsrc + (int64_t)j * p.head_js + (int64_t)ct * p.head_ns);
    }
    wgmma_wait<0>();
    mbar_arrive(empty0 + 8 * prev);
    if (EPI == 4 || EPI == 6) named_bar_sync<CONSUMER_BAR, CONSUMER_THREADS>();
    const int r0 = m0 + cw * 64 + (warp & 3) * 16 + (lane >> 2), cl = (lane & 3) * 2;
    float* C = g.C + (int64_t)grp * g.c_gs + (int64_t)r0 * g.ldc + cl;
    const int64_t c8 = (int64_t)8 * g.ldc;
    const float* bias = (EPI == 1 || (EPI == 3 && g.bias)) ? g.bias + (int64_t)grp * g.bias_gs + cl : nullptr;
    const float* mask = (EPI == 2 || (EPI == 3 && g.mask)) ? g.mask + (int64_t)grp * g.mask_gs + (int64_t)r0 * g.ldmask + cl : nullptr;
    const int64_t m8 = (int64_t)8 * g.ldmask;
    const uint32_t* mbits = (EPI == 5 || EPI == 6) ? g.mask_bits + (int64_t)grp * g.mask_bits_gs + (int64_t)r0 * (BN / 32) : nullptr;
    uint32_t word0 = 0, word1 = 0;
#pragma unroll
    for (int c = 0; c < BN / 8; ++c) {
      float v00 = acc[4 * c], v01 = acc[4 * c + 1], v10 = acc[4 * c + 2], v11 = acc[4 * c + 3];
      const int col = 8 * c, bit = (c & 3) * 8 + cl;
      if (EPI == 5 || EPI == 6) {
        if ((c & 3) == 0) { word0 = __ldg(mbits + (c >> 2)); word1 = __ldg(mbits + 8 * (BN / 32) + (c >> 2)); }
        v00 = (word0 >> bit) & 1u ? v00 : 0.f; v01 = (word0 >> (bit + 1)) & 1u ? v01 : 0.f;
        v10 = (word1 >> bit) & 1u ? v10 : 0.f; v11 = (word1 >> (bit + 1)) & 1u ? v11 : 0.f;
      }
      if (EPI == 4) {
        const float2 b = *reinterpret_cast<const float2*>(head_s + col + cl);
        v00 = fmaxf(v00 + b.x, 0.f); v01 = fmaxf(v01 + b.y, 0.f); v10 = fmaxf(v10 + b.x, 0.f); v11 = fmaxf(v11 + b.y, 0.f);
        if (g.bits_out) {
          if ((c & 3) == 0) word0 = word1 = 0;
          word0 |= (v00 > 0.f ? 1u : 0u) << bit | (v01 > 0.f ? 1u : 0u) << (bit + 1);
          word1 |= (v10 > 0.f ? 1u : 0u) << bit | (v11 > 0.f ? 1u : 0u) << (bit + 1);
          if ((c & 3) == 3) {
            word0 |= __shfl_xor_sync(0xffffffffu, word0, 1); word0 |= __shfl_xor_sync(0xffffffffu, word0, 2);
            word1 |= __shfl_xor_sync(0xffffffffu, word1, 1); word1 |= __shfl_xor_sync(0xffffffffu, word1, 2);
            if ((lane & 3) == 0) {
              uint32_t* bo = g.bits_out + (int64_t)grp * g.bits_out_gs + (int64_t)r0 * (BN / 32) + (c >> 2);
              bo[0] = word0;
              bo[8 * (BN / 32)] = word1;
            }
          }
        }
      }
      if (EPI == 4 || EPI == 6) {
        acc[4 * c] = v00; acc[4 * c + 1] = v01; acc[4 * c + 2] = v10; acc[4 * c + 3] = v11;
        if (!p.store_c) continue;
      }
      if (EPI == 1) {
        const float2 b = __ldg(reinterpret_cast<const float2*>(bias + col));
        v00 = fmaxf(v00 + b.x, 0.f); v01 = fmaxf(v01 + b.y, 0.f); v10 = fmaxf(v10 + b.x, 0.f); v11 = fmaxf(v11 + b.y, 0.f);
      } else if (EPI == 2) {
        const float2 ma = __ldg(reinterpret_cast<const float2*>(mask + col)), mb = __ldg(reinterpret_cast<const float2*>(mask + m8 + col));
        v00 = ma.x > 0.f ? v00 : 0.f; v01 = ma.y > 0.f ? v01 : 0.f; v10 = mb.x > 0.f ? v10 : 0.f; v11 = mb.y > 0.f ? v11 : 0.f;
      } else if (EPI == 3) {
        if (bias) {
          const float2 b = __ldg(reinterpret_cast<const float2*>(bias + col));
          v00 += b.x; v01 += b.y; v10 += b.x; v11 += b.y;
        }
        if (g.act >= 0) { v00 = act_apply(v00, g.act); v01 = act_apply(v01, g.act); v10 = act_apply(v10, g.act); v11 = act_apply(v11, g.act); }
        if (mask) {
          const float2 ma = __ldg(reinterpret_cast<const float2*>(mask + col)), mb = __ldg(reinterpret_cast<const float2*>(mask + m8 + col));
          v00 *= act_grad_from_output(ma.x, g.mask_act); v01 *= act_grad_from_output(ma.y, g.mask_act);
          v10 *= act_grad_from_output(mb.x, g.mask_act); v11 *= act_grad_from_output(mb.y, g.mask_act);
        }
      }
      *reinterpret_cast<float2*>(C + col) = make_float2(v00, v01);
      *reinterpret_cast<float2*>(C + c8 + col) = make_float2(v10, v11);
    }
    if (EPI == 4 || EPI == 6) {
      float* ho = p.head_out + (int64_t)grp * p.head_out_gs + (int64_t)r0 * p.head_n;
      const float* hb = p.head_b ? p.head_b + (int64_t)grp * p.head_gs : nullptr;
#pragma unroll 1
      for (int j = 0; j < HEAD_MAX; ++j) {
        if (j < p.head_n) {
          float s0 = 0.f, s1 = 0.f;
#pragma unroll
          for (int c = 0; c < BN / 8; ++c) {
            const float2 w = *reinterpret_cast<const float2*>(head_s + BN + j * BN + 8 * c + cl);
            s0 = fmaf(acc[4 * c], w.x, s0); s0 = fmaf(acc[4 * c + 1], w.y, s0);
            s1 = fmaf(acc[4 * c + 2], w.x, s1); s1 = fmaf(acc[4 * c + 3], w.y, s1);
          }
          s0 += __shfl_xor_sync(0xffffffffu, s0, 1); s0 += __shfl_xor_sync(0xffffffffu, s0, 2);
          s1 += __shfl_xor_sync(0xffffffffu, s1, 1); s1 += __shfl_xor_sync(0xffffffffu, s1, 2);
          if ((lane & 3) == 0) {
            const float b = hb ? __ldg(hb + j) : 0.f;
            ho[j] = s0 + b;
            ho[(int64_t)8 * p.head_n + j] = s1 + b;
          }
        }
      }
    }
  }
}


__global__ void colsum_kernel(const float* __restrict__ A, int64_t a_gs, int a_gdiv, int lda, int K, int M, float* __restrict__ out, int64_t out_gs) {
  const int g = blockIdx.y, m = blockIdx.x * blockDim.x + threadIdx.x;
  if (m >= M) return;
  const float* a = A + (int64_t)(g / a_gdiv) * a_gs + m;
  float s = 0.f;
  for (int k = 0; k < K; ++k) s += a[(int64_t)k * lda];
  out[(int64_t)g * out_gs + m] = s;
}

}

bool tc_gemm_eligible(const GemmArgs& a) {
  auto al16 = [](const void* p) { return (reinterpret_cast<uintptr_t>(p) & 15) == 0; };
  if (a.M % BM != 0 || a.N != BN || a.K % BK != 0 || a.accumulate) return false;
  if (a.a_kmajor == 0 && a.b_kmajor != 0) return false;
  if (!al16(a.A) || !al16(a.B) || !al16(a.C) || a.lda % 4 || a.ldb % 4 || a.ldc % 4 || a.a_gs % 4 || a.b_gs % 4 || a.c_gs % 4) return false;
  if (a.bias && (!al16(a.bias) || a.bias_gs % 4)) return false;
  if (a.mask && (!al16(a.mask) || a.ldmask % 4 || a.mask_gs % 4)) return false;
  return true;
}

template <int EPI, bool FUSE = false>
int tc_set_attr() {
  IL_CUDA(cudaFuncSetAttribute(tc_gemm_kernel<EPI, FUSE>, cudaFuncAttributeMaxDynamicSharedMemorySize, smem_bytes(FUSE)));
  return 0;
}

int tc_gemm_init() {
  IL_TRY((tc_set_attr<0>())); IL_TRY((tc_set_attr<1>())); IL_TRY((tc_set_attr<2>())); IL_TRY((tc_set_attr<3>())); IL_TRY((tc_set_attr<4>()));
  IL_TRY((tc_set_attr<4, true>())); IL_TRY((tc_set_attr<5>())); IL_TRY((tc_set_attr<6>()));
  return 0;
}

template <int EPI, bool FUSE = false>
static int tc_launch(il_handle* h, TcParams& p, cudaStream_t stream) {
  const GemmArgs& a = p.g;
  p.tiles_m = a.M / BM;
  const int tiles = a.G * p.tiles_m, wave = h->sm_count >= p.tiles_m ? h->sm_count / p.tiles_m * p.tiles_m : h->sm_count;
  IL_LAUNCH(h, (tc_gemm_kernel<EPI, FUSE>), tiles < wave ? tiles : wave, THREADS, smem_bytes(FUSE), stream, p);
  return 0;
}

bool tc_head_fusable(const il_handle* h, const GemmArgs& a, int head_n) {
  return h->gemm_mode != IL_GEMM_FP32 && tc_gemm_eligible(a) && a.bias && a.act == IL_ACT_RELU && !a.mask && !a.colsum && head_n >= 1 && head_n <= HEAD_MAX;
}

bool tc_l1_fusable(const il_handle* h, const GemmArgs& a, int x_k) {
  return h->tc_fuse_l1 && tc_gemm_eligible(a) && x_k >= 1 && x_k <= L1_MAXK && a.K <= L1_ROWS && a.a_kmajor;
}

int launch_tc_gemm_head(il_handle* h, const GemmArgs& a, const float* head_w, const float* head_b, int64_t head_gs, int head_n, float* head_out, int64_t head_out_gs, int store_c,
                        cudaStream_t stream, const TcFuseL1* l1) {
  IL_CHECK(tc_head_fusable(h, a, head_n), "tc_gemm_head: not fusable");
  TcParams p{};
  p.g = a;
  p.split = h->gemm_mode == IL_GEMM_TF32X3 ? 1 : 0;
  p.head_w = head_w; p.head_b = head_b; p.head_out = head_out; p.head_gs = head_gs; p.head_out_gs = head_out_gs; p.head_n = head_n; p.store_c = store_c;
  p.head_js = BN; p.head_ns = 1;
  double bytes = gemm_algorithmic_bytes(a, store_c != 0) + 4.0 * a.G * (double)a.M * head_n, flops = 2.0 * a.M * a.N * a.K * a.G;
  if (l1) {
    IL_CHECK(tc_l1_fusable(h, a, l1->x_k), "tc_gemm_head: first layer not fusable (K0=%d)", l1->x_k);
    IL_CHECK(l1->x && l1->w1 && l1->b1 && (reinterpret_cast<uintptr_t>(l1->b1) & 15) == 0 && l1->gs % 4 == 0, "tc_gemm_head: bad first-layer buffers");
    IL_CHECK(!l1->store || ((reinterpret_cast<uintptr_t>(l1->store) & 15) == 0 && l1->store_gs % 4 == 0), "tc_gemm_head: unaligned hidden store");
    p.l1 = *l1;
    const double gx = (a.G + l1->x_gdiv - 1) / l1->x_gdiv;
    bytes += -4.0 * a.G * (double)a.M * a.K + 4.0 * (gx * a.M * l1->x_k + (double)a.G * a.K * (l1->x_k + 1)) + (l1->store ? 4.0 * a.G * (double)a.M * a.K : 0.0);
    flops += 2.0 * a.G * (double)a.M * a.K * l1->x_k;
  }
  auto run = [&]() { return l1 ? tc_launch<4, true>(h, p, stream) : tc_launch<4>(h, p, stream); };
  if (h->profiling) {
    ProfiledLaunch pl;
    IL_TRY(profile_open(h, &pl, flops, bytes, stream));
    const int rc = run();
    IL_TRY(profile_close(h, &pl, stream));
    return rc;
  }
  return run();
}

bool tc_dx_head_fusable(const il_handle* h, const GemmArgs& a, int head_n) {
  return h->gemm_mode != IL_GEMM_FP32 && a.M >= 128 && a.K >= 128 && tc_gemm_eligible(a) && a.mask_bits && !a.mask && !a.bias && a.act < 0 && !a.colsum && a.mask_act == IL_ACT_RELU &&
         head_n >= 1 && head_n <= HEAD_MAX;
}
int launch_tc_gemm_dx_head(il_handle* h, const GemmArgs& a, const float* w, int64_t w_gs, int w_ns, int head_n, float* out, int64_t out_gs, cudaStream_t stream) {
  IL_CHECK(tc_dx_head_fusable(h, a, head_n), "tc_gemm_dx_head: not fusable");
  TcParams p{};
  p.g = a;
  p.split = h->gemm_mode == IL_GEMM_TF32X3 ? 1 : 0;
  p.head_w = w; p.head_b = nullptr; p.head_out = out; p.head_gs = w_gs; p.head_out_gs = out_gs; p.head_n = head_n; p.store_c = 0;
  p.head_js = 1; p.head_ns = w_ns;
  const double bytes = gemm_algorithmic_bytes(a, false) + 4.0 * a.G * (double)a.M * head_n, flops = 2.0 * a.M * a.N * a.K * a.G;
  if (h->profiling) {
    ProfiledLaunch pl;
    IL_TRY(profile_open(h, &pl, flops, bytes, stream));
    const int rc = tc_launch<6>(h, p, stream);
    IL_TRY(profile_close(h, &pl, stream));
    return rc;
  }
  return tc_launch<6>(h, p, stream);
}

int launch_tc_gemm(il_handle* h, const GemmArgs& a, cudaStream_t stream) {
  IL_CHECK(tc_gemm_eligible(a), "tc_gemm: shape/layout not eligible (M=%d N=%d K=%d)", a.M, a.N, a.K);
  TcParams p{};
  p.g = a;
  p.split = h->gemm_mode == IL_GEMM_TF32X3 ? 1 : 0;
  const bool bits = a.mask_bits != nullptr;
  IL_CHECK(!bits || (!a.bias && a.act < 0 && a.mask_act == IL_ACT_RELU), "tc_gemm: sign-bit masks are the ReLU derivative of a plain product");
  if (bits) p.g.mask = nullptr;
  const bool plain = !a.bias && a.act < 0 && !a.mask && !bits;
  const bool bias_relu = a.bias && a.act == IL_ACT_RELU && !a.mask;
  const bool mask_relu = !a.bias && a.act < 0 && a.mask && a.mask_act == IL_ACT_RELU && !bits;
  if (bits) IL_TRY(tc_launch<5>(h, p, stream));
  else if (plain) IL_TRY(tc_launch<0>(h, p, stream));
  else if (bias_relu) IL_TRY(tc_launch<1>(h, p, stream));
  else if (mask_relu) IL_TRY(tc_launch<2>(h, p, stream));
  else IL_TRY(tc_launch<3>(h, p, stream));
  if (a.colsum) {
    dim3 cg((a.M + 127) / 128, a.G);
    IL_LAUNCH(h, colsum_kernel, cg, 128, 0, stream, a.A, a.a_gs, a.a_gdiv, a.lda, a.K, a.M, a.colsum, a.colsum_gs);
  }
  return 0;
}
```

Baseline: 86530.

## Fuse SAC critic loss gradient and head backward into the hidden-layer GEMM epilogue

Result: faster. 88560, median of 6 (+2.3%).

```diff
diff --git a/imitation-learning_b200/csrc/api.cu b/imitation-learning_b200/csrc/api.cu
--- a/imitation-learning_b200/csrc/api.cu
+++ b/imitation-learning_b200/csrc/api.cu
@@ -46,6 +46,8 @@
     h->gail_tiled = (gt && gt[0] == '0') ? 0 : 1;
     const char* fl = getenv("IL_TC_FUSE_L1");
     h->tc_fuse_l1 = (fl && fl[0] == '1') ? 1 : 0;
+    const char* cf = getenv("IL_CRITIC_FUSED");
+    h->critic_fused = (cf && cf[0] == '0') ? 0 : 1;
     const char* th = getenv("IL_THIN_HOIST");
     h->thin_hoist = (th && th[0] == '0') ? 0 : 1;
   }
@@ -80,6 +82,7 @@
   else if (!strcmp(name, "gail_tiled")) h->gail_tiled = value;
   else if (!strcmp(name, "adam_tma")) h->adam_tma = value;
   else if (!strcmp(name, "head_fused")) h->head_fused = value;
+  else if (!strcmp(name, "critic_fused")) h->critic_fused = value;
   else if (!strcmp(name, "mask_bits")) h->mask_bits = value;
   else if (!strcmp(name, "first_layer_fast")) h->first_layer_fast = value;
   else if (!strcmp(name, "wide_tn")) h->wide_tn = value;
diff --git a/imitation-learning_b200/csrc/common.cuh b/imitation-learning_b200/csrc/common.cuh
--- a/imitation-learning_b200/csrc/common.cuh
+++ b/imitation-learning_b200/csrc/common.cuh
@@ -28,6 +28,7 @@
   int adam_tma;
   int gail_tiled;
   int tc_fuse_l1;
+  int critic_fused;
   long long launches;
   int profiling;
   std::vector<ProfiledLaunch> profiled;
@@ -205,9 +206,18 @@
   float* store;
   int64_t store_gs;
 };
+struct TcLossGrad {
+  const float* y;
+  int64_t y_gs;
+  int y_gdiv;
+  const float* w;
+  int64_t w_gs;
+  int w_gdiv, w_ld;
+  float* part;
+};
 bool tc_head_fusable(const il_handle* h, const GemmArgs& a, int head_n);
 bool tc_l1_fusable(const il_handle* h, const GemmArgs& a, int x_k);
 bool tc_dx_head_fusable(const il_handle* h, const GemmArgs& a, int head_n);
 int launch_tc_gemm_dx_head(il_handle* h, const GemmArgs& a, const float* w, int64_t w_gs, int w_ns, int head_n, float* out, int64_t out_gs, cudaStream_t stream);
 int launch_tc_gemm_head(il_handle* h, const GemmArgs& a, const float* head_w, const float* head_b, int64_t head_gs, int head_n, float* head_out, int64_t head_out_gs, int store_c,
-                        cudaStream_t stream, const TcFuseL1* l1 = nullptr);
+                        cudaStream_t stream, const TcFuseL1* l1 = nullptr, const TcLossGrad* lg = nullptr);
diff --git a/imitation-learning_b200/csrc/mlp.cu b/imitation-learning_b200/csrc/mlp.cu
--- a/imitation-learning_b200/csrc/mlp.cu
+++ b/imitation-learning_b200/csrc/mlp.cu
@@ -54,36 +54,54 @@
   return ws;
 }
 
-int mlp_forward(il_handle* h, const il_mlp* m, int G, int n, MatView X, MlpActs& acts, float* out, int64_t out_gs, int ld_out, cudaStream_t stream, int keep) {
+static GemmArgs mlp_layer_args(const il_mlp* m, const MlpOffsets& o, int G, int n, const MatView& X, const MlpActs& acts, float* out, int64_t out_gs, int ld_out, int l) {
+  const int L = m->n_layers;
+  GemmArgs a{};
+  if (l == 0) { a.A = X.ptr; a.a_gs = X.gs; a.a_gdiv = X.gdiv; a.lda = X.ld; }
+  else { a.A = acts.hid[l - 1]; a.a_gs = (int64_t)n * m->dims[l]; a.a_gdiv = 1; a.lda = m->dims[l]; }
+  a.a_kmajor = 1;
+  a.B = m->params + o.w[l]; a.b_gs = m->stride; a.b_gdiv = 1; a.ldb = m->dims[l]; a.b_kmajor = 1;
+  a.bias = m->params + o.b[l]; a.bias_gs = m->stride;
+  if (l == L - 1) { a.C = out; a.c_gs = out_gs; a.ldc = ld_out; a.act = -1; }
+  else { a.C = acts.hid[l]; a.c_gs = (int64_t)n * m->dims[l + 1]; a.ldc = m->dims[l + 1]; a.act = m->activation; }
+  a.M = n; a.N = m->dims[l + 1]; a.K = m->dims[l]; a.G = G;
+  return a;
+}
+
+static bool head_backward_eligible(const il_mlp* m, int n, int64_t grad_stride) {
+  const int L = m->n_layers, H = m->dims[L - 1], Nh = m->dims[L];
+  return m->activation == IL_ACT_RELU && Nh <= HB_MAXN && H % 4 == 0 && n <= 1024 && grad_stride % 4 == 0 && m->stride % 4 == 0;
+}
+
+bool mlp_lossgrad_fusable(const il_handle* h, const il_mlp* m, int G, int n, const MlpActs& acts, int64_t grad_stride) {
+  const int L = m->n_layers;
+  if (!h->critic_fused || !h->head_fused || h->tc_fuse_l1 || L != 3 || m->dims[L] != 1 || !head_backward_eligible(m, n, grad_stride)) return false;
+  const GemmArgs a = mlp_layer_args(m, mlp_offsets(m->dims, L), G, n, MatView{}, acts, nullptr, n, 1, L - 2);
+  return tc_head_fusable(h, a, 1);
+}
+
+int mlp_forward(il_handle* h, const il_mlp* m, int G, int n, MatView X, MlpActs& acts, float* out, int64_t out_gs, int ld_out, cudaStream_t stream, int keep,
+                const TcLossGrad* lg) {
   const MlpOffsets o = mlp_offsets(m->dims, m->n_layers);
   const int L = m->n_layers;
   const bool keep_hidden = keep != MLP_KEEP_NONE;
   const bool want_bits = h->mask_bits && keep_hidden && m->activation == IL_ACT_RELU;
   for (int l = 0; l < IL_MAX_LAYERS; ++l) acts.bits_valid[l] = false;
-  auto layer_args = [&](int l) {
-    GemmArgs a{};
-    if (l == 0) { a.A = X.ptr; a.a_gs = X.gs; a.a_gdiv = X.gdiv; a.lda = X.ld; }
-    else { a.A = acts.hid[l - 1]; a.a_gs = (int64_t)n * m->dims[l]; a.a_gdiv = 1; a.lda = m->dims[l]; }
-    a.a_kmajor = 1;
-    a.B = m->params + o.w[l]; a.b_gs = m->stride; a.b_gdiv = 1; a.ldb = m->dims[l]; a.b_kmajor = 1;
-    a.bias = m->params + o.b[l]; a.bias_gs = m->stride;
-    if (l == L - 1) { a.C = out; a.c_gs = out_gs; a.ldc = ld_out; a.act = -1; }
-    else { a.C = acts.hid[l]; a.c_gs = (int64_t)n * m->dims[l + 1]; a.ldc = m->dims[l + 1]; a.act = m->activation; }
-    a.M = n; a.N = m->dims[l + 1]; a.K = m->dims[l]; a.G = G;
-    return a;
-  };
+  auto layer_args = [&](int l) { return mlp_layer_args(m, o, G, n, X, acts, out, out_gs, ld_out, l); };
+  IL_CHECK(!lg || (mlp_lossgrad_fusable(h, m, G, n, acts, m->stride) && out_gs == n && ld_out == 1), "mlp_forward: the loss-gradient epilogue does not apply to this net");
   const bool head_shape = L >= 2 && m->activation == IL_ACT_RELU && ld_out == m->dims[L] && out_gs == (int64_t)n * m->dims[L];
   for (int l = 0; l < L; ++l) {
     if (head_shape && l == L - 2) {
       GemmArgs a = layer_args(l);
       if (tc_head_fusable(h, a, m->dims[L])) {
-        const bool bits = want_bits && keep == MLP_KEEP_MASKS && acts.bits[l] && m->dims[L] <= HB_MAXN;
+        const bool bits = !lg && want_bits && keep == MLP_KEEP_MASKS && acts.bits[l] && m->dims[L] <= HB_MAXN;
         if (bits) { a.bits_out = acts.bits[l]; a.bits_out_gs = (int64_t)n * (m->dims[l + 1] / 32); acts.bits_valid[l] = true; }
-        IL_TRY(launch_tc_gemm_head(h, a, m->params + o.w[L - 1], m->params + o.b[L - 1], m->stride, m->dims[L], out, out_gs, keep_hidden && !bits ? 1 : 0, stream));
+        IL_TRY(launch_tc_gemm_head(h, a, m->params + o.w[L - 1], m->params + o.b[L - 1], m->stride, m->dims[L], out, out_gs, (keep_hidden && !bits) || lg ? 1 : 0, stream,
+                                   nullptr, lg));
         return 0;
       }
     }
-    if (head_shape && l == 0 && L == 3) {
+    if (head_shape && l == 0 && L == 3 && !lg) {
       GemmArgs a1 = layer_args(1);
       a1.A = nullptr; a1.a_gs = 0; a1.a_gdiv = 1; a1.lda = m->dims[1];
       if (tc_head_fusable(h, a1, m->dims[L]) && tc_l1_fusable(h, a1, m->dims[0])) {
@@ -105,19 +123,14 @@
   return 0;
 }
 
-static bool head_backward_eligible(const il_mlp* m, int n, int64_t grad_stride) {
-  const int L = m->n_layers, H = m->dims[L - 1], Nh = m->dims[L];
-  return m->activation == IL_ACT_RELU && Nh <= HB_MAXN && H % 4 == 0 && n <= 1024 && grad_stride % 4 == 0 && m->stride % 4 == 0;
-}
-
 int mlp_backward(il_handle* h, const il_mlp* m, int G, int n, MatView X, const MlpActs& acts, MatView dOut, float* grads, int64_t grad_stride,
-                 float* dX, int64_t dx_gs, int ld_dx, int dx_col0, int dx_cols, float* tmpA, float* tmpB, cudaStream_t stream) {
+                 float* dX, int64_t dx_gs, int ld_dx, int dx_col0, int dx_cols, float* tmpA, float* tmpB, cudaStream_t stream, bool from_last_hidden) {
   const MlpOffsets o = mlp_offsets(m->dims, m->n_layers);
   const int L = m->n_layers;
   MatView dZ = dOut;
   float* next_tmp = tmpA;
-  bool bias_done = false;
-  for (int l = L - 1; l >= 0; --l) {
+  bool bias_done = from_last_hidden;
+  for (int l = from_last_hidden ? L - 2 : L - 1; l >= 0; --l) {
     MatView Xin = l == 0 ? X : MatView{acts.hid[l - 1], (int64_t)n * m->dims[l], 1, m->dims[l]};
     if (l == L - 1 && l > 0 && grads && h->head_fused && head_backward_eligible(m, n, grad_stride)) {
       HeadBwdArgs a{};
diff --git a/imitation-learning_b200/csrc/mlp.cuh b/imitation-learning_b200/csrc/mlp.cuh
--- a/imitation-learning_b200/csrc/mlp.cuh
+++ b/imitation-learning_b200/csrc/mlp.cuh
@@ -19,10 +19,11 @@
 char* mlp_acts_carve(const il_mlp* m, int G, int n, char* ws, MlpActs* acts);
 
 int mlp_forward(il_handle* h, const il_mlp* m, int G, int n, MatView X, MlpActs& acts, float* out, int64_t out_gs, int ld_out,
-                cudaStream_t stream, int keep = MLP_KEEP_ALL);
+                cudaStream_t stream, int keep = MLP_KEEP_ALL, const TcLossGrad* lg = nullptr);
+bool mlp_lossgrad_fusable(const il_handle* h, const il_mlp* m, int G, int n, const MlpActs& acts, int64_t grad_stride);
 
 int mlp_backward(il_handle* h, const il_mlp* m, int G, int n, MatView X, const MlpActs& acts, MatView dOut, float* grads, int64_t grad_stride,
-                 float* dX, int64_t dx_gs, int ld_dx, int dx_col0, int dx_cols, float* tmpA, float* tmpB, cudaStream_t stream);
+                 float* dX, int64_t dx_gs, int ld_dx, int dx_col0, int dx_cols, float* tmpA, float* tmpB, cudaStream_t stream, bool from_last_hidden = false);
 
 int mlp_small_forward(il_handle* h, const il_mlp* m, int G, int n, MatView X, float* out, cudaStream_t stream, int tanh_first = 0);
 int mlp_max_hidden(const il_mlp* m);
diff --git a/imitation-learning_b200/csrc/sac.cu b/imitation-learning_b200/csrc/sac.cu
--- a/imitation-learning_b200/csrc/sac.cu
+++ b/imitation-learning_b200/csrc/sac.cu
@@ -24,8 +24,15 @@
   y[i] = __fadd_rn(tr[off_reward], __fmul_rn(__fmul_rn(__fsub_rn(1.f, tr[off_terminal]), discount), tv));
 }
 
+struct CriticHeadGrads {
+  const float* part;
+  int tiles, H;
+  float* grads;
+  int64_t stride, w, b, b_prev;
+};
+
 __global__ void sac_critic_lossgrad_kernel(const float* __restrict__ q, const float* __restrict__ y, const float* __restrict__ rows, int64_t rs, int row, int off_weight,
-                                           float* __restrict__ dq, float* __restrict__ out_q, float* __restrict__ out_losses, int B) {
+                                           float* __restrict__ dq, float* __restrict__ out_q, float* __restrict__ out_losses, int B, const CriticHeadGrads hg) {
   __shared__ float red[32];
   const int r = blockIdx.x;
   const float invB = 1.f / (float)B;
@@ -37,14 +44,34 @@
     const float d1 = __fsub_rn(q1, yy), d2 = __fsub_rn(q2, yy);
     l1 += w * d1 * d1;
     l2 += w * d2 * d2;
-    const float c = __fmul_rn(invB, w);
-    dq[((int64_t)2 * r) * B + b] = __fmul_rn(c, __fmul_rn(2.f, d1));
-    dq[((int64_t)2 * r + 1) * B + b] = __fmul_rn(c, __fmul_rn(2.f, d2));
+    if (dq) {
+      const float c = __fmul_rn(invB, w);
+      dq[((int64_t)2 * r) * B + b] = __fmul_rn(c, __fmul_rn(2.f, d1));
+      dq[((int64_t)2 * r + 1) * B + b] = __fmul_rn(c, __fmul_rn(2.f, d2));
+    }
     if (out_q) out_q[(int64_t)r * B + b] = fminf(q1, q2);
   }
   l1 = block_sum(l1, red);
   l2 = block_sum(l2, red);
   if (threadIdx.x == 0 && out_losses) out_losses[r * 3 + 0] = l1 * invB + l2 * invB;
+  if (!hg.part) return;
+  const int64_t pt = 2 * (int64_t)hg.H + 4;
+  for (int g = 2 * r; g < 2 * r + 2; ++g) {
+    const float* part = hg.part + (int64_t)g * hg.tiles * pt;
+    float* gr = hg.grads + (int64_t)g * hg.stride;
+    for (int c = threadIdx.x; c <= hg.H; c += blockDim.x) {
+      if (c < hg.H) {
+        float sw = part[c], sz = part[hg.H + c];
+        for (int t = 1; t < hg.tiles; ++t) { sw += part[t * pt + c]; sz += part[t * pt + hg.H + c]; }
+        gr[hg.w + c] = sw;
+        gr[hg.b_prev + c] = sz;
+      } else {
+        float s = part[2 * hg.H];
+        for (int t = 1; t < hg.tiles; ++t) s += part[t * pt + 2 * hg.H];
+        gr[hg.b] = s;
+      }
+    }
+  }
 }
 
 __global__ void sac_actor_loss_kernel(const float* __restrict__ q, const float* __restrict__ lp_new, const float* __restrict__ log_alpha, const float* __restrict__ rows,
@@ -156,7 +183,7 @@
 
 struct SacWs {
   MlpActs actor_acts, critic_acts;
-  float *head, *q, *xn, *y, *lp_next, *dq, *dxa, *dhead, *tmpA, *tmpB, *g_actor, *g_critic;
+  float *head, *q, *xn, *y, *lp_next, *dq, *dxa, *dhead, *tmpA, *tmpB, *g_actor, *g_critic, *critic_part;
   int64_t bytes;
 };
 
@@ -187,6 +214,8 @@
   w.tmpB = take((int64_t)2 * R * B * hmax);
   w.g_actor = take((int64_t)R * a->actor.stride);
   w.g_critic = take((int64_t)2 * R * a->critic.stride);
+  const int Lc = a->critic.n_layers;
+  w.critic_part = take((int64_t)2 * R * ((B + 127) / 128) * (2 * (int64_t)a->critic.dims[Lc - 1] + 4));
   w.bytes = p - base;
   return w;
 }
@@ -241,10 +270,21 @@
   }
   IL_TRY(mlp_forward(h, &a->target, 2 * R, B, MatView{w.xn, (int64_t)B * d, 2, d}, w.critic_acts, w.q, (int64_t)B, 1, st, false));
   IL_LAUNCH(h, sac_target_kernel, ew, 128, 0, st, w.q, w.lp_next, a->log_alpha, rows, rs, row, L.reward, L.terminal, av, a->discount, a->discount_r, w.y, R, B);
-  IL_TRY(mlp_forward(h, &a->critic, 2 * R, B, MatView{rows + L.state, rs, 2, row}, w.critic_acts, w.q, (int64_t)B, 1, st));
-  IL_LAUNCH(h, sac_critic_lossgrad_kernel, R, 256, 0, st, w.q, w.y, rows, rs, row, L.weight, w.dq, a->out_q_values, a->out_losses, B);
-  IL_TRY(mlp_backward(h, &a->critic, 2 * R, B, MatView{rows + L.state, rs, 2, row}, w.critic_acts, MatView{w.dq, (int64_t)B, 1, 1}, w.g_critic, a->critic.stride, nullptr, 0,
-                      0, 0, 0, w.tmpA, w.tmpB, st));
+  const MatView Xc{rows + L.state, rs, 2, row};
+  if (mlp_lossgrad_fusable(h, &a->critic, 2 * R, B, w.critic_acts, a->critic.stride)) {
+    const int Lc = a->critic.n_layers, H = a->critic.dims[Lc - 1];
+    const MlpOffsets oc = mlp_offsets(a->critic.dims, Lc);
+    const TcLossGrad lg{w.y, (int64_t)B, 2, rows + L.weight, rs, 2, row, w.critic_part};
+    IL_TRY(mlp_forward(h, &a->critic, 2 * R, B, Xc, w.critic_acts, w.q, (int64_t)B, 1, st, MLP_KEEP_ALL, &lg));
+    const CriticHeadGrads hg{w.critic_part, B / 128, H, w.g_critic, a->critic.stride, oc.w[Lc - 1], oc.b[Lc - 1], oc.b[Lc - 2]};
+    IL_LAUNCH(h, sac_critic_lossgrad_kernel, R, 256, 0, st, w.q, w.y, rows, rs, row, L.weight, nullptr, a->out_q_values, a->out_losses, B, hg);
+    IL_TRY(mlp_backward(h, &a->critic, 2 * R, B, Xc, w.critic_acts, MatView{w.critic_acts.hid[Lc - 2], (int64_t)B * H, 1, H}, w.g_critic, a->critic.stride, nullptr, 0, 0, 0, 0,
+                        w.tmpA, w.tmpB, st, true));
+  } else {
+    IL_TRY(mlp_forward(h, &a->critic, 2 * R, B, Xc, w.critic_acts, w.q, (int64_t)B, 1, st));
+    IL_LAUNCH(h, sac_critic_lossgrad_kernel, R, 256, 0, st, w.q, w.y, rows, rs, row, L.weight, w.dq, a->out_q_values, a->out_losses, B, CriticHeadGrads{});
+    IL_TRY(mlp_backward(h, &a->critic, 2 * R, B, Xc, w.critic_acts, MatView{w.dq, (int64_t)B, 1, 1}, w.g_critic, a->critic.stride, nullptr, 0, 0, 0, 0, w.tmpA, w.tmpB, st));
+  }
   IL_TRY(launch_adam(h, a->critic.params, w.g_critic, &a->critic_opt, (int64_t)2 * R * a->critic.stride, st, a->target.params, a->polyak_factor, a->polyak_r));
   IL_TRY(mlp_forward(h, &a->actor, R, B, MatView{rows + L.state, rs, 1, row}, w.actor_acts, w.head, (int64_t)B * 2 * A, 2 * A, st));
   {
diff --git a/imitation-learning_b200/csrc/tc_gemm.cu b/imitation-learning_b200/csrc/tc_gemm.cu
--- a/imitation-learning_b200/csrc/tc_gemm.cu
+++ b/imitation-learning_b200/csrc/tc_gemm.cu
@@ -29,8 +29,13 @@
 constexpr int l1_off(bool fuse) { return head_off(fuse) + HEAD_BYTES; }
 constexpr int BAR_BYTES = 64;
 static_assert(2 * N_STAGES * 8 <= BAR_BYTES && BAR_BYTES + 512 - 16 <= 1024, "tc_gemm: mbarrier area");
-constexpr int smem_bytes(bool fuse) { return 1024 + l1_off(fuse) + (fuse ? L1_W_BYTES + L1_B_BYTES + L1_X_BYTES : 0); }
-static_assert(smem_bytes(false) <= 227 * 1024 && smem_bytes(true) <= 227 * 1024, "tc_gemm: shared memory over the 227 KB per-CTA limit");
+constexpr int CONSUMER_WARPS = CONSUMER_THREADS / 32;
+constexpr int LG_RED_BYTES = CONSUMER_WARPS * 2 * BN * 4, LG_ROW_BYTES = 2 * BM * 4, LG_BYTES = LG_RED_BYTES + LG_ROW_BYTES + CONSUMER_WARPS * 4;
+constexpr int LG_PART = 2 * BN + 4;
+constexpr int smem_bytes(bool fuse, bool lg = false) {
+  return 1024 + l1_off(fuse) + (fuse ? L1_W_BYTES + L1_B_BYTES + L1_X_BYTES : lg ? LG_BYTES : 0);
+}
+static_assert(smem_bytes(false) <= 227 * 1024 && smem_bytes(true) <= 227 * 1024 && smem_bytes(false, true) <= 227 * 1024, "tc_gemm: shared memory over the 227 KB per-CTA limit");
 
 __device__ __forceinline__ uint32_t smem_u32(const void* p) { return (uint32_t)__cvta_generic_to_shared(p); }
 __device__ __forceinline__ void fence_proxy_async() { asm volatile("fence.proxy.async.shared::cta;" ::: "memory"); }
@@ -138,6 +143,7 @@
   int head_n, store_c;
   int head_js, head_ns;
   TcFuseL1 l1;
+  TcLossGrad lg;
 };
 
 template <int EPI, bool FUSE = false>
@@ -150,6 +156,10 @@
   const uint32_t w1s = stage0 + l1_off(FUSE), b1s = w1s + L1_W_BYTES, xs = b1s + L1_B_BYTES;
   auto a_slot = [&](int q) { return a0s + (uint32_t)(q % A_STAGES) * (uint32_t)a_slot_bytes(FUSE); };
   const bool a_km = FUSE || p.g.a_kmajor != 0;
+  constexpr bool HEAD = EPI == 4 || EPI == 6 || EPI == 7;
+  float* lg_red = reinterpret_cast<float*>(smem + l1_off(FUSE));
+  float* lg_y = lg_red + CONSUMER_WARPS * 2 * BN;
+  float* lg_dq = lg_y + 2 * BM;
 
   const int tid = threadIdx.x, warp = tid >> 5, lane = tid & 31, wg = tid >> 7;
   const GemmArgs& g = p.g;
@@ -341,6 +351,11 @@
   for (int i = 0; i < my_tiles; ++i) {
 #pragma unroll
     for (int j = 0; j < 128; ++j) acc[j] = 0.f;
+    float lg_row = 0.f;
+    if (EPI == 7) {
+      const int t = tile_of(i), grp = t / tiles_m, m = (t % tiles_m) * BM + ct % BM;
+      lg_row = ct < BM ? __ldg(p.lg.y + (int64_t)(grp / p.lg.y_gdiv) * p.lg.y_gs + m) : __ldg(p.lg.w + (int64_t)(grp / p.lg.w_gdiv) * p.lg.w_gs + (int64_t)m * p.lg.w_ld);
+    }
     int prev = 0;
     auto step = [&](int kb, uint32_t (&f)[2][BK / 8][4]) {
       mbar_wait(full0 + 8 * s, ph);
@@ -358,17 +373,18 @@
     }
 
     const int t = tile_of(i), grp = t / tiles_m, m0 = (t % tiles_m) * BM;
-    if (EPI == 4 || EPI == 6) {
+    if (HEAD) {
       named_bar_sync<CONSUMER_BAR, CONSUMER_THREADS>();
       const float* wsrc = p.head_w + (int64_t)grp * p.head_gs;
-      if (EPI == 4) head_s[ct] = __ldg(g.bias + (int64_t)grp * g.bias_gs + ct);
+      if (EPI == 4 || EPI == 7) head_s[ct] = __ldg(g.bias + (int64_t)grp * g.bias_gs + ct);
+      if (EPI == 7) lg_y[ct] = lg_row;
 #pragma unroll
       for (int j = 0; j < HEAD_MAX; ++j)
         if (j < p.head_n) head_s[BN + j * BN + ct] = __ldg(wsrc + (int64_t)j * p.head_js + (int64_t)ct * p.head_ns);
     }
     wgmma_wait<0>();
     mbar_arrive(empty0 + 8 * prev);
-    if (EPI == 4 || EPI == 6) named_bar_sync<CONSUMER_BAR, CONSUMER_THREADS>();
+    if (HEAD) named_bar_sync<CONSUMER_BAR, CONSUMER_THREADS>();
     const int r0 = m0 + cw * 64 + (warp & 3) * 16 + (lane >> 2), cl = (lane & 3) * 2;
     float* C = g.C + (int64_t)grp * g.c_gs + (int64_t)r0 * g.ldc + cl;
     const int64_t c8 = (int64_t)8 * g.ldc;
@@ -386,7 +402,7 @@
         v00 = (word0 >> bit) & 1u ? v00 : 0.f; v01 = (word0 >> (bit + 1)) & 1u ? v01 : 0.f;
         v10 = (word1 >> bit) & 1u ? v10 : 0.f; v11 = (word1 >> (bit + 1)) & 1u ? v11 : 0.f;
       }
-      if (EPI == 4) {
+      if (EPI == 4 || EPI == 7) {
         const float2 b = *reinterpret_cast<const float2*>(head_s + col + cl);
         v00 = fmaxf(v00 + b.x, 0.f); v01 = fmaxf(v01 + b.y, 0.f); v10 = fmaxf(v10 + b.x, 0.f); v11 = fmaxf(v11 + b.y, 0.f);
         if (g.bits_out) {
@@ -404,9 +420,9 @@
           }
         }
       }
-      if (EPI == 4 || EPI == 6) {
+      if (HEAD) {
         acc[4 * c] = v00; acc[4 * c + 1] = v01; acc[4 * c + 2] = v10; acc[4 * c + 3] = v11;
-        if (!p.store_c) continue;
+        if (EPI == 7 || !p.store_c) continue;
       }
       if (EPI == 1) {
         const float2 b = __ldg(reinterpret_cast<const float2*>(bias + col));
@@ -429,27 +445,90 @@
       *reinterpret_cast<float2*>(C + col) = make_float2(v00, v01);
       *reinterpret_cast<float2*>(C + c8 + col) = make_float2(v10, v11);
     }
+    auto head_dot = [&](int j, float& s0, float& s1) {
+      s0 = 0.f; s1 = 0.f;
+#pragma unroll
+      for (int c = 0; c < BN / 8; ++c) {
+        const float2 w = *reinterpret_cast<const float2*>(head_s + BN + j * BN + 8 * c + cl);
+        s0 = fmaf(acc[4 * c], w.x, s0); s0 = fmaf(acc[4 * c + 1], w.y, s0);
+        s1 = fmaf(acc[4 * c + 2], w.x, s1); s1 = fmaf(acc[4 * c + 3], w.y, s1);
+      }
+      s0 += __shfl_xor_sync(0xffffffffu, s0, 1); s0 += __shfl_xor_sync(0xffffffffu, s0, 2);
+      s1 += __shfl_xor_sync(0xffffffffu, s1, 1); s1 += __shfl_xor_sync(0xffffffffu, s1, 2);
+    };
     if (EPI == 4 || EPI == 6) {
       float* ho = p.head_out + (int64_t)grp * p.head_out_gs + (int64_t)r0 * p.head_n;
       const float* hb = p.head_b ? p.head_b + (int64_t)grp * p.head_gs : nullptr;
 #pragma unroll 1
       for (int j = 0; j < HEAD_MAX; ++j) {
         if (j < p.head_n) {
-          float s0 = 0.f, s1 = 0.f;
-#pragma unroll
-          for (int c = 0; c < BN / 8; ++c) {
-            const float2 w = *reinterpret_cast<const float2*>(head_s + BN + j * BN + 8 * c + cl);
-            s0 = fmaf(acc[4 * c], w.x, s0); s0 = fmaf(acc[4 * c + 1], w.y, s0);
-            s1 = fmaf(acc[4 * c + 2], w.x, s1); s1 = fmaf(acc[4 * c + 3], w.y, s1);
-          }
-          s0 += __shfl_xor_sync(0xffffffffu, s0, 1); s0 += __shfl_xor_sync(0xffffffffu, s0, 2);
-          s1 += __shfl_xor_sync(0xffffffffu, s1, 1); s1 += __shfl_xor_sync(0xffffffffu, s1, 2);
+          float s0, s1;
+          head_dot(j, s0, s1);
           if ((lane & 3) == 0) {
             const float b = hb ? __ldg(hb + j) : 0.f;
             ho[j] = s0 + b;
             ho[(int64_t)8 * p.head_n + j] = s1 + b;
           }
         }
+      }
+    }
+    if (EPI == 7) {
+      float s0, s1;
+      head_dot(0, s0, s1);
+      const float hb = __ldg(p.head_b + (int64_t)grp * p.head_gs), q0 = s0 + hb, q1 = s1 + hb;
+      if ((lane & 3) == 0) {
+        float* ho = p.head_out + (int64_t)grp * p.head_out_gs + r0;
+        ho[0] = q0;
+        ho[8] = q1;
+      }
+      const int lr = r0 - m0;
+      const float invB = 1.f / (float)g.M;
+      const float dq0 = __fmul_rn(__fmul_rn(invB, lg_y[BM + lr]), __fmul_rn(2.f, __fsub_rn(q0, lg_y[lr])));
+      const float dq1 = __fmul_rn(__fmul_rn(invB, lg_y[BM + lr + 8]), __fmul_rn(2.f, __fsub_rn(q1, lg_y[lr + 8])));
+      const int cwarp = ct >> 5, g8 = lane >> 2;
+      float* rw = lg_red + cwarp * 2 * BN + ((g8 >> 1) & 1) * BN + 8 * (g8 >> 2) + cl + (g8 & 1);
+#pragma unroll
+      for (int c = 0; c < BN / 8; c += 2) {
+        float v[8];
+#pragma unroll
+        for (int i = 0; i < 2; ++i) {
+          const int col = 8 * (c + i);
+          const float2 w = *reinterpret_cast<const float2*>(head_s + BN + col + cl);
+          const float h00 = acc[4 * (c + i)], h01 = acc[4 * (c + i) + 1], h10 = acc[4 * (c + i) + 2], h11 = acc[4 * (c + i) + 3];
+          float z00 = fmaf(dq0, w.x, 0.f), z01 = fmaf(dq0, w.y, 0.f), z10 = fmaf(dq1, w.x, 0.f), z11 = fmaf(dq1, w.y, 0.f);
+          z00 = h00 > 0.f ? z00 : 0.f; z01 = h01 > 0.f ? z01 : 0.f; z10 = h10 > 0.f ? z10 : 0.f; z11 = h11 > 0.f ? z11 : 0.f;
+          *reinterpret_cast<float2*>(C + col) = make_float2(z00, z01);
+          *reinterpret_cast<float2*>(C + c8 + col) = make_float2(z10, z11);
+          v[4 * i] = fmaf(dq1, h10, dq0 * h00); v[4 * i + 1] = fmaf(dq1, h11, dq0 * h01);
+          v[4 * i + 2] = z00 + z10; v[4 * i + 3] = z01 + z11;
+        }
+#pragma unroll
+        for (int lv = 2; lv >= 0; --lv) {
+          const int half = 1 << lv;
+          const bool upper = (lane >> (2 + lv)) & 1;
+#pragma unroll
+          for (int k = 0; k < half; ++k) {
+            const float send = upper ? v[k] : v[k + half], keep = upper ? v[k + half] : v[k];
+            v[k] = keep + __shfl_xor_sync(0xffffffffu, send, 4 << lv);
+          }
+        }
+        rw[8 * c] = v[0];
+      }
+      float dqs = dq0 + dq1;
+      dqs += __shfl_xor_sync(0xffffffffu, dqs, 4); dqs += __shfl_xor_sync(0xffffffffu, dqs, 8); dqs += __shfl_xor_sync(0xffffffffu, dqs, 16);
+      if (lane == 0) lg_dq[cwarp] = dqs;
+      named_bar_sync<CONSUMER_BAR, CONSUMER_THREADS>();
+      float sw = 0.f, sz = 0.f;
+#pragma unroll
+      for (int q8 = 0; q8 < CONSUMER_WARPS; ++q8) { sw += lg_red[q8 * 2 * BN + ct]; sz += lg_red[q8 * 2 * BN + BN + ct]; }
+      float* part = p.lg.part + ((int64_t)grp * tiles_m + t % tiles_m) * LG_PART;
+      part[ct] = sw;
+      part[BN + ct] = sz;
+      if (ct == 0) {
+        float s = 0.f;
+#pragma unroll
+        for (int q8 = 0; q8 < CONSUMER_WARPS; ++q8) s += lg_dq[q8];
+        part[2 * BN] = s;
       }
     }
   }
@@ -479,13 +558,13 @@
 
 template <int EPI, bool FUSE = false>
 int tc_set_attr() {
-  IL_CUDA(cudaFuncSetAttribute(tc_gemm_kernel<EPI, FUSE>, cudaFuncAttributeMaxDynamicSharedMemorySize, smem_bytes(FUSE)));
+  IL_CUDA(cudaFuncSetAttribute(tc_gemm_kernel<EPI, FUSE>, cudaFuncAttributeMaxDynamicSharedMemorySize, smem_bytes(FUSE, EPI == 7)));
   return 0;
 }
 
 int tc_gemm_init() {
   IL_TRY((tc_set_attr<0>())); IL_TRY((tc_set_attr<1>())); IL_TRY((tc_set_attr<2>())); IL_TRY((tc_set_attr<3>())); IL_TRY((tc_set_attr<4>()));
-  IL_TRY((tc_set_attr<4, true>())); IL_TRY((tc_set_attr<5>())); IL_TRY((tc_set_attr<6>()));
+  IL_TRY((tc_set_attr<4, true>())); IL_TRY((tc_set_attr<5>())); IL_TRY((tc_set_attr<6>())); IL_TRY((tc_set_attr<7>()));
   return 0;
 }
 
@@ -494,7 +573,7 @@
   const GemmArgs& a = p.g;
   p.tiles_m = a.M / BM;
   const int tiles = a.G * p.tiles_m, wave = h->sm_count >= p.tiles_m ? h->sm_count / p.tiles_m * p.tiles_m : h->sm_count;
-  IL_LAUNCH(h, (tc_gemm_kernel<EPI, FUSE>), tiles < wave ? tiles : wave, THREADS, smem_bytes(FUSE), stream, p);
+  IL_LAUNCH(h, (tc_gemm_kernel<EPI, FUSE>), tiles < wave ? tiles : wave, THREADS, smem_bytes(FUSE, EPI == 7), stream, p);
   return 0;
 }
 
@@ -507,8 +586,9 @@
 }
 
 int launch_tc_gemm_head(il_handle* h, const GemmArgs& a, const float* head_w, const float* head_b, int64_t head_gs, int head_n, float* head_out, int64_t head_out_gs, int store_c,
-                        cudaStream_t stream, const TcFuseL1* l1) {
+                        cudaStream_t stream, const TcFuseL1* l1, const TcLossGrad* lg) {
   IL_CHECK(tc_head_fusable(h, a, head_n), "tc_gemm_head: not fusable");
+  IL_CHECK(!lg || (!l1 && head_n == 1 && store_c && head_b && lg->y && lg->w && lg->part), "tc_gemm_head: the loss-gradient epilogue needs one head unit, its bias and no fused first layer");
   TcParams p{};
   p.g = a;
   p.split = h->gemm_mode == IL_GEMM_TF32X3 ? 1 : 0;
@@ -524,7 +604,11 @@
     bytes += -4.0 * a.G * (double)a.M * a.K + 4.0 * (gx * a.M * l1->x_k + (double)a.G * a.K * (l1->x_k + 1)) + (l1->store ? 4.0 * a.G * (double)a.M * a.K : 0.0);
     flops += 2.0 * a.G * (double)a.M * a.K * l1->x_k;
   }
-  auto run = [&]() { return l1 ? tc_launch<4, true>(h, p, stream) : tc_launch<4>(h, p, stream); };
+  if (lg) {
+    p.lg = *lg;
+    bytes += 8.0 * a.G * (double)a.M + 4.0 * a.G * (a.M / BM) * LG_PART;
+  }
+  auto run = [&]() { return l1 ? tc_launch<4, true>(h, p, stream) : lg ? tc_launch<7>(h, p, stream) : tc_launch<4>(h, p, stream); };
   if (h->profiling) {
     ProfiledLaunch pl;
     IL_TRY(profile_open(h, &pl, flops, bytes, stream));
```
